# cserteGT3/RANSAC.jl

Measured on AMD Instinct MI355X. Metric: candidates_scored_per_sec, higher is better.
Workload: dtype f64; 1 GPU; cfg3: 10M-point 40-primitive cloud, 30% outliers, r=32 subsets, B=4096 candidates/GPU/step; points=10000000, subset_points=312500, score_mode=f64, parallelism=candidate-sharded x1, int32 sum all-reduce

## Files before the change

### include/ransac_hip_diag.h

```cpp
#ifndef RANSAC_HIP_DIAG_H
#define RANSAC_HIP_DIAG_H

#include "ransac_hip.h"

#ifdef __cplusplus
extern "C" {
#endif

int rh_dbg_cls_audit(rh_cloud *c, const rh_shape *shapes, int32_t b, const rh_params *p, double *out );
int rh_dbg_cls_soundness(rh_cloud *c, const rh_shape *shapes, int32_t b, const rh_params *p, uint64_t *out );
int rh_dbg_cls_soundness_tiles(rh_cloud *c, const rh_shape *shapes, int32_t b, const rh_params *p, uint64_t *out );
int rh_dbg_cls_soundness_nsig(rh_cloud *c, const rh_shape *shapes, int32_t b, const rh_params *p, uint64_t *out );
int rh_dbg_nsig(const rh_shape *shape, const rh_params *p, double M, double Nm, double Ln, int f32, uint32_t *mask_out ,
                const double *dirs, int64_t ndirs, int32_t *cells_out);
int rh_dbg_group_boxes(rh_cloud *c, double *out, int64_t cap, int64_t *ngroups_out);
int rh_dbg_kd_shape(int64_t s, int aligned, int64_t *info_out , int64_t *nodes_out, int64_t node_cap, int64_t *splits_out,
                    int64_t split_cap, int64_t *leaves_out, int64_t leaf_cap);
int rh_dbg_plane_order(rh_cloud *c, int64_t *info_out , double *sub_out, double *pl_out, int32_t *src_out, float *gb32_out,
                       uint32_t *gm32_out, uint64_t *en_out);
int rh_dbg_cylbox(const rh_shape *shape, const rh_params *p, double M, double Nm, int f32, const double *boxes, int64_t n,
                  uint8_t *skip_out, uint8_t *ball_out, float *fields_out );
int rh_dbg_cls_round(const rh_shape *shape, const rh_params *p, double M, double Nm, int f32, int64_t n, const double *xyz,
                     const double *nrm, float *ua_out, float *ub_out, float *rec_out , double *dbg4_out );
int rh_dbg_books2(const float *u2, int64_t nseq, int32_t *sure_count_out, uint64_t *sure_word_out, uint64_t *und_word_out,
                  uint8_t *any_und_out);
int rh_dbg_cls_u2(const rh_shape *shape, const rh_params *p, double M, double Nm, int f32, int64_t n, const double *xyz,
                  const double *nrm, float *u_out, float *u2_out, float *rec_out );
int rh_dbg_conebox(const rh_shape *shape, const rh_params *p, double M, double Nm, int f32, const double *boxes, int64_t n,
                   uint8_t *skip_out, float *fields_out );
int rh_dbg_cls_cone(const rh_shape *shape, const rh_params *p, double M, double Nm, int f32, int64_t n, const double *xyz,
                    const double *nrm, int device, float *ua_out, float *ub_out, uint8_t *near_out, float *rec_out ,
                    double *dbg4_out );
int rh_dbg_oct_search_selftest(int64_t n, uint64_t seed, int64_t queries, int64_t *mismatches);

int rh_dbg_enabled_events(const uint8_t *events, int64_t nseq, int32_t len, uint16_t *answers);

int rh_dbg_s4_stats(rh_cloud *c, int mode, uint64_t *out );

typedef struct { int64_t slot; int32_t level; int32_t pad; rh_shape shape; } rh_dbg_cand;
int rh_dbg_sample_fit(rh_cloud *c, const rh_params *p, uint64_t seed, int64_t k0, int32_t n_iters, const double *P_or_null,
                      int32_t rank, int32_t world, rh_dbg_cand *out, int32_t cap, int32_t *n_out, uint64_t *draws_out,
                      int32_t *gave_up_out, int32_t *info_out );

int rh_dbg_wave_keys(const uint32_t *keys, const uint8_t *act, const int32_t *slot, int32_t n, int32_t nslots, int u32, int device,
                     int32_t *sum_out , int32_t *minlead_out , int32_t *scal_out );

#ifdef __cplusplus
}
#endif
#endif
```

### ransac.jl_amd/_lib.py

```python
import ctypes as C
import os

_HERE = os.path.dirname(os.path.abspath(__file__))
SO_PATH = os.path.join(_HERE, "libransac_hip.so")
SO_PATH_DIAG = os.path.join(_HERE, "libransac_hip_diag.so")
OPTION_UNSET = -(1 << 63)
SCORE_PATH = {"auto": 0, "brute": 1, "groups": 2}
REFIT_PATH = {"auto": 0, "scan": 1, "culled": 2}

PLANE, SPHERE, CYLINDER, CONE = 0, 1, 2, 3
KIND_NAMES = {PLANE: "plane", SPHERE: "sphere", CYLINDER: "cylinder", CONE: "cone"}
SCORE_INT64_WRAP, SCORE_F64 = 0, 1
S_LENGTHC, S_ALLCAND, S_NOFMINSET = 1, 2, 3
RH_OK, RH_E_INVALID, RH_E_NODEVICE, RH_E_NOMEM, RH_E_CAPACITY, RH_E_INTERNAL = 0, -1, -2, -3, -4, -5


class Shape(C.Structure):
    _fields_ = [("kind", C.c_int32), ("outwards", C.c_int32), ("v", C.c_double * 10)]


class Params(C.Structure):
    _fields_ = [
        ("eps", C.c_double * 4), ("alpha", C.c_double * 4), ("cos_alpha", C.c_double * 4),
        ("collin_threshold", C.c_double), ("parallelthrdeg", C.c_double), ("cos_parallelthr", C.c_double),
# ... 200 lines not shown
    "rh_octree_info": (C.c_int, [_vp, _i32p, _i32p, _i32p]),
    "rh_octree_findleaf": (C.c_int, [_vp, _dp, _i32p]),
    "rh_octree_getnthcell": (C.c_int, [_vp, C.c_int32, C.c_int32, _i32p]),
    "rh_octree_node_info": (C.c_int, [_vp, C.c_int32, _dp, _dp, _i32p, _i32p, _i32p, C.POINTER(C.c_int64)]),
    "rh_octree_node_points": (C.c_int, [_vp, C.c_int32, C.POINTER(C.c_int64), C.c_int64]),
    "rh_octree_cell_enabled": (C.c_int, [_vp, _vp, C.c_int32, C.POINTER(C.c_int64), C.c_int64, C.POINTER(C.c_int64)]),
    "rh_set_option": (C.c_int, [_vp, C.c_char_p, C.c_int64]),
    "rh_get_option": (C.c_int, [_vp, C.c_char_p, _i64p, _i32p]),
    "rh_score_launch_info": (C.c_int, [_vp, C.POINTER(C.c_int32)]),
    "rh_last_list_launch_ms": (C.c_int, [_vp, C.POINTER(C.c_float)]),
    "rh_build_variant": (C.c_int, []),
    "rh_cloud_create_ms": (C.c_int, [_vp, _dp]),
    "rh_comm_unique_id": (C.c_int, [_vp]),
    "rh_comm_create": (C.c_int, [_vp, C.c_int32, C.c_int32, _vp, C.POINTER(_vp)]),
    "rh_comm_destroy": (C.c_int, [_vp]),
    "rh_score_batch_allreduce_dev": (C.c_int, [_vp, _vp, _vp, C.c_int32, C.c_int32, C.c_int32, _pp, _vp]),
    "rh_comm_fence": (C.c_int, [_vp, _vp]),
    "rh_comm_sync": (C.c_int, [_vp]),
    "rh_shape_extents": (C.c_int, [_vp, _sp, C.c_int32, _i64p, _i64p, C.POINTER(Extent)]),
    "rh_shape_extents_dev": (C.c_int, [_vp, _vp, C.c_int32, _vp, _vp, C.c_int64, _vp]),
    "rh_result_extents": (C.c_int, [_vp, C.POINTER(Result), C.POINTER(Extent)]),
    "rh_assign_points": (C.c_int, [_dp, _dp, C.c_int64, _sp, C.c_int32, _pp, C.c_int32, C.c_int, _i32p, _dp, _i64p, _i64p, _i64p]),
    "rh_assign_points_f32": (C.c_int, [C.POINTER(C.c_float), C.POINTER(C.c_float), C.c_int64, _sp, C.c_int32, _pp, C.c_int32, C.c_int,
                                       _i32p, _dp, _i64p, _i64p, _i64p]),
    "rh_cloud_assign": (C.c_int, [_vp, _sp, C.c_int32, _pp, C.c_int32, _i32p, _dp, _i64p, _i64p, _i64p]),
    "rh_cloud_assign_dev": (C.c_int, [_vp, _vp, C.c_int32, _pp, C.c_int32, _vp, _vp, _vp, _vp, _vp]),
    "rh_estimate_normals": (C.c_int, [_dp, C.c_int64, C.POINTER(NormalsParams), _dp, C.c_int, _dp, _dp, _i32p]),
    "rh_estimate_normals_f32": (C.c_int, [C.POINTER(C.c_float), C.c_int64, C.POINTER(NormalsParams), C.POINTER(C.c_float),
                                          C.c_int, C.POINTER(C.c_float), C.POINTER(C.c_float), _i32p]),
    "rh_cluster": (C.c_int, [_dp, C.c_int64, C.POINTER(ClusterParams), C.c_int, _i32p, _u8p, C.c_int64, _i64p, _i64p, _i64p, _i64p,
                             C.POINTER(ClusterStats)]),
    "rh_cluster_f32": (C.c_int, [C.POINTER(C.c_float), C.c_int64, C.POINTER(ClusterParams), C.c_int, _i32p, _u8p, C.c_int64, _i64p,
                                 _i64p, _i64p, _i64p, C.POINTER(ClusterStats)]),
    "rh_segment_smooth": (C.c_int, [_dp, _dp, _dp, C.c_int64, C.POINTER(SegmentParams), C.c_int, _i32p, _u8p, C.c_int64, _i64p, _i64p,
                                    _i64p, _i64p, C.POINTER(SegmentStats)]),
    "rh_segment_smooth_f32": (C.c_int, [C.POINTER(C.c_float), C.POINTER(C.c_float), C.POINTER(C.c_float), C.c_int64,
                                        C.POINTER(SegmentParams), C.c_int, _i32p, _u8p, C.c_int64, _i64p, _i64p, _i64p, _i64p,
                                        C.POINTER(SegmentStats)]),
    "rh_orient_normals": (C.c_int, [_dp, _dp, C.c_int64, C.POINTER(OrientParams), C.c_int, _dp, _i32p, _i32p, C.POINTER(OrientStats)]),
    "rh_orient_normals_f32": (C.c_int, [C.POINTER(C.c_float), C.POINTER(C.c_float), C.c_int64, C.POINTER(OrientParams), C.c_int,
                                        C.POINTER(C.c_float), _i32p, _i32p, C.POINTER(OrientStats)]),
    "rh_voxel_downsample": (C.c_int, [_dp, _dp, C.c_int64, C.POINTER(VoxelParams), C.c_int, _dp, _dp, _i64p, _i32p, C.c_int64,
                                      _i32p, _i64p, _i64p]),
    "rh_voxel_downsample_f32": (C.c_int, [C.POINTER(C.c_float), C.POINTER(C.c_float), C.c_int64, C.POINTER(VoxelParams), C.c_int,
                                          C.POINTER(C.c_float), C.POINTER(C.c_float), _i64p, _i32p, C.c_int64, _i32p, _i64p, _i64p]),
    "rh_knn": (C.c_int, [_dp, C.c_int64, C.c_int32, C.c_double, C.c_int, _i32p, _dp, _i32p]),
    "rh_knn_f32": (C.c_int, [C.POINTER(C.c_float), C.c_int64, C.c_int32, C.c_double, C.c_int, _i32p, _dp, _i32p]),
    "rh_knn_query": (C.c_int, [_dp, C.c_int64, _dp, C.c_int64, C.c_int32, C.c_double, C.c_int, _i32p, _dp, _i32p]),
    "rh_knn_query_f32": (C.c_int, [C.POINTER(C.c_float), C.c_int64, C.POINTER(C.c_float), C.c_int64, C.c_int32, C.c_double, C.c_int,
                                   _i32p, _dp, _i32p]),
    "rh_cloud_distance": (C.c_int, [_dp, _dp, C.c_int64, _dp, C.c_int64, C.POINTER(DistanceParams), C.c_int, _dp, _i32p,
                                    C.POINTER(DistanceStats)]),
    "rh_cloud_distance_f32": (C.c_int, [C.POINTER(C.c_float), C.POINTER(C.c_float), C.c_int64, C.POINTER(C.c_float), C.c_int64,
                                        C.POINTER(DistanceParams), C.c_int, _dp, _i32p, C.POINTER(DistanceStats)]),
    "rh_register": (C.c_int, [_dp, _dp, C.c_int64, _dp, C.c_int64, C.POINTER(RegisterParams), _dp, C.c_int, _dp,
                              C.POINTER(RegisterResult), _i32p, _dp]),
    "rh_register_f32": (C.c_int, [C.POINTER(C.c_float), C.POINTER(C.c_float), C.c_int64, C.POINTER(C.c_float), C.c_int64,
                                  C.POINTER(RegisterParams), _dp, C.c_int, _dp, C.POINTER(RegisterResult), _i32p, _dp]),
    "rh_describe": (C.c_int, [_dp, _dp, C.c_int64, C.c_int32, C.c_double, C.c_int, _u16p, _i32p]),
    "rh_describe_f32": (C.c_int, [C.POINTER(C.c_float), C.POINTER(C.c_float), C.c_int64, C.c_int32, C.c_double, C.c_int, _u16p,
                                  _i32p]),
    "rh_match_features": (C.c_int, [_u16p, C.c_int64, _u16p, C.c_int64, C.c_int32, C.c_int, _i32p, _u32p]),
    "rh_register_global": (C.c_int, [_dp, C.c_int64, _dp, C.c_int64, _i32p, _i32p, C.c_int64, C.POINTER(GlobalParams), _i32p,
                                     C.c_int, _dp, C.POINTER(GlobalResult), _i32p]),
    "rh_register_global_f32": (C.c_int, [C.POINTER(C.c_float), C.c_int64, C.POINTER(C.c_float), C.c_int64, _i32p, _i32p, C.c_int64,
                                         C.POINTER(GlobalParams), _i32p, C.c_int, _dp, C.POINTER(GlobalResult), _i32p]),
    "rh_remove_outliers": (C.c_int, [_dp, C.c_int64, C.POINTER(OutlierParams), C.c_int, _u8p, _i32p, C.c_int64, _i64p, _dp,
                                     C.POINTER(OutlierStats)]),
    "rh_remove_outliers_f32": (C.c_int, [C.POINTER(C.c_float), C.c_int64, C.POINTER(OutlierParams), C.c_int, _u8p, _i32p,
                                         C.c_int64, _i64p, _dp, C.POINTER(OutlierStats)]),
}

class DbgCand(C.Structure):
    _fields_ = [("slot", C.c_int64), ("level", C.c_int32), ("pad", C.c_int32), ("shape", Shape)]


DIAG_SIGNATURES = {
    "rh_dbg_sample_fit": (C.c_int, [_vp, _pp, C.c_uint64, C.c_int64, C.c_int32, _dp, C.c_int32, C.c_int32, C.POINTER(DbgCand),
                                    C.c_int32, _i32p, _u64p, _i32p, _i32p]),
    "rh_dbg_cls_audit": (C.c_int, [_vp, _sp, C.c_int32, _pp, _dp]),
    "rh_dbg_cls_soundness": (C.c_int, [_vp, _sp, C.c_int32, _pp, C.POINTER(C.c_uint64)]),
    "rh_dbg_cls_soundness_tiles": (C.c_int, [_vp, _sp, C.c_int32, _pp, C.POINTER(C.c_uint64)]),
    "rh_dbg_cls_soundness_nsig": (C.c_int, [_vp, _sp, C.c_int32, _pp, C.POINTER(C.c_uint64)]),
    "rh_dbg_nsig": (C.c_int, [_sp, _pp, C.c_double, C.c_double, C.c_double, C.c_int, C.POINTER(C.c_uint32), _dp, C.c_int64, _i32p]),
    "rh_dbg_group_boxes": (C.c_int, [_vp, _dp, C.c_int64, C.POINTER(C.c_int64)]),
    "rh_dbg_kd_shape": (C.c_int, [C.c_int64, C.c_int, _i64p, _i64p, C.c_int64, _i64p, C.c_int64, _i64p, C.c_int64]),
    "rh_dbg_plane_order": (C.c_int, [_vp, _i64p, _dp, _dp, _i32p, C.POINTER(C.c_float), C.POINTER(C.c_uint32), _u64p]),
    "rh_dbg_cylbox": (C.c_int, [_sp, _pp, C.c_double, C.c_double, C.c_int, _dp, C.c_int64, C.POINTER(C.c_uint8), C.POINTER(C.c_uint8), C.POINTER(C.c_float)]),
    "rh_dbg_cls_round": (C.c_int, [_sp, _pp, C.c_double, C.c_double, C.c_int, C.c_int64, _dp, _dp, C.POINTER(C.c_float), C.POINTER(C.c_float),
                                   C.POINTER(C.c_float), _dp]),
    "rh_dbg_books2": (C.c_int, [C.POINTER(C.c_float), C.c_int64, _i32p, _u64p, _u64p, _u8p]),
    "rh_dbg_cls_u2": (C.c_int, [_sp, _pp, C.c_double, C.c_double, C.c_int, C.c_int64, _dp, _dp, C.POINTER(C.c_float), C.POINTER(C.c_float),
                                C.POINTER(C.c_float)]),
    "rh_dbg_conebox": (C.c_int, [_sp, _pp, C.c_double, C.c_double, C.c_int, _dp, C.c_int64, C.POINTER(C.c_uint8), C.POINTER(C.c_float)]),
    "rh_dbg_cls_cone": (C.c_int, [_sp, _pp, C.c_double, C.c_double, C.c_int, C.c_int64, _dp, _dp, C.c_int, C.POINTER(C.c_float),
                                  C.POINTER(C.c_float), C.POINTER(C.c_uint8), C.POINTER(C.c_float), _dp]),
    "rh_dbg_oct_search_selftest": (C.c_int, [C.c_int64, C.c_uint64, C.c_int64, C.POINTER(C.c_int64)]),
    "rh_dbg_enabled_events": (C.c_int, [_u8p, C.c_int64, C.c_int32, C.POINTER(C.c_uint16)]),
    "rh_dbg_s4_stats": (C.c_int, [_vp, C.c_int, C.POINTER(C.c_uint64)]),
    "rh_dbg_wave_keys": (C.c_int, [C.POINTER(C.c_uint32), _u8p, _i32p, C.c_int32, C.c_int32, C.c_int, C.c_int, _i32p, _i32p, _i32p]),
}

_libs = {}


def variant():
    v = os.environ.get("RH_LIB_VARIANT", "product")
    if v not in ("product", "diag"):
        raise RuntimeError("RH_LIB_VARIANT=%r: expected 'product' or 'diag'" % v)
    return v


def _share_torch_hip_runtime():
    import sys
    if "torch" in sys.modules or os.environ.get("RH_SYSTEM_HIP"):
        return
    try:
        import importlib.util
        spec = importlib.util.find_spec("torch")
        if spec is None or not spec.submodule_search_locations:
            return
        path = os.path.join(list(spec.submodule_search_locations)[0], "lib", "libamdhip64.so")
        if os.path.exists(path):
            C.CDLL(path, mode=C.RTLD_GLOBAL)
    except (ImportError, OSError, ValueError):
        pass


def lib(which=None):
    which = which or variant()
    L = _libs.get(which)
    if L is None:
        path = SO_PATH if which == "product" else SO_PATH_DIAG
        if os.environ.get("RH_LIB_PATH"):
            path = os.environ["RH_LIB_PATH"]
        if not os.path.exists(path):
            raise RuntimeError(
                "%s is missing: the HIP extension has not been built and this package has no CPU "
                "fallback (build it with ransac.jl_amd/build.py)" % path)
        _share_torch_hip_runtime()
        L = C.CDLL(path)
        sigs = dict(SIGNATURES)
        if which == "diag":
            sigs.update(DIAG_SIGNATURES)
        for name, (res, args) in sigs.items():
            f = getattr(L, name, None)
            if f is None and os.environ.get("RH_LIB_PATH"):
                continue
            if f is None:
                raise AttributeError("%s does not export %s" % (path, name))
            f.restype = res
            f.argtypes = args
        if L.rh_build_variant() != (1 if which == "diag" else 0):
            raise RuntimeError("%s is not the %s build" % (path, which))
        _libs[which] = L
    return L


def check(rc):
    if rc != RH_OK:
        raise RansacHipError(rc, lib().rh_last_error().decode("utf-8", "replace"))
    return rc
```

### ransac.jl_amd/csrc/boxes32.hip

```cpp
#include "rh_internal.h"
#include "score_device.h"
#include "score4_device.h"
#include "score4_shared.h"

namespace {

using namespace rhdev;
using namespace rh4;

__global__ void gb32_kernel(const double *__restrict__ gb, int64_t gstride, int64_t ngroups, float *__restrict__ out)
{
    const int64_t g = (int64_t)blockIdx.x * blockDim.x + threadIdx.x;
    if (g >= ngroups) return;
    const double c[3] = { gb[g], gb[gstride + g], gb[2 * gstride + g] };
    const double h[3] = { gb[3 * gstride + g], gb[4 * gstride + g], gb[5 * gstride + g] };
    float o[8];
    box_to_f32(c, h, o);
#pragma unroll
    for (int k = 0; k < 8; k++) out[g * 8 + k] = o[k];
}

__global__ void st32_kernel(const double *__restrict__ gb, int64_t gstride, int64_t ngroups, int k_groups, int64_t nst, float *__restrict__ out)
{
    const int64_t st = (int64_t)blockIdx.x * blockDim.x + threadIdx.x;
    if (st >= nst) return;
    double lo[3] = { __builtin_inf(), __builtin_inf(), __builtin_inf() }, hi[3] = { -__builtin_inf(), -__builtin_inf(), -__builtin_inf() };
    bool bad = false;
    for (int64_t g = st * k_groups; g < (st + 1) * k_groups && g < ngroups; g++)
#pragma unroll
        for (int k = 0; k < 3; k++) {
            const double cc = gb[k * gstride + g], hh = gb[(3 + k) * gstride + g];
            bad |= !(fabs(cc) < __builtin_inf()) || !(fabs(hh) < __builtin_inf());
            lo[k] = fmin(lo[k], cc - hh);
            hi[k] = fmax(hi[k], cc + hh);
        }
    double c3[3], h3[3];
#pragma unroll
    for (int k = 0; k < 3; k++) {
        c3[k] = 0.5 * lo[k] + 0.5 * hi[k];
        h3[k] = fmax(hi[k] - c3[k], c3[k] - lo[k]) * 1.000000000001 + (fabs(lo[k]) + fabs(hi[k])) * 1e-15;
        bad |= !(fabs(c3[k]) < __builtin_inf()) || !(h3[k] < __builtin_inf());
    }
    float o[8];
    box_to_f32(c3, h3, o);
#pragma unroll
    for (int k = 0; k < 8; k++) out[st * 8 + k] = bad ? __builtin_nanf("") : o[k];
}

__global__ void __launch_bounds__(256)
nsig_kernel(const double *__restrict__ pts, int64_t stride, int64_t s, int64_t ngroups, uint32_t *__restrict__ out, unsigned long long *__restrict__ maxlen)
{
    __shared__ uint32_t m[4][4];
    const int lane = threadIdx.x & 63, wv = threadIdx.x >> 6;
    const int64_t g = (int64_t)blockIdx.x * 4 + wv;
    if (lane < 4) m[wv][lane] = 0u;
    __syncthreads();
    const int64_t i = g * 64 + lane;
    double len = 0.0;
    if (g < ngroups && i < s) {
        const double nx = pts[3 * stride + i], ny = pts[4 * stride + i], nz = pts[5 * stride + i];
        uint32_t w[3];
        nsig_point_bits(nx, ny, nz, w);
        if (w[0] != 0u) atomicOr(&m[wv][0], w[0]);
        if (w[1] != 0u) atomicOr(&m[wv][1], w[1]);
        if (w[2] != 0u) atomicOr(&m[wv][2], w[2]);
        const double l = sqrt((nx * nx + ny * ny) + nz * nz);
        if (l < __builtin_inf()) len = l;
    }
    unsigned long long lb = __builtin_bit_cast(unsigned long long, len);
    for (int off = 32; off > 0; off >>= 1) { const unsigned long long v = __shfl_down(lb, off); lb = v > lb ? v : lb; }
    if (lane == 0 && lb != 0ULL) atomicMax(maxlen, lb);
    __syncthreads();
    if (g < ngroups && lane < 4) out[g * 4 + lane] = m[wv][lane];
}

__global__ void nsig_st_kernel(const uint32_t *__restrict__ gm, int64_t ngroups, int k_groups, int64_t nst, uint32_t *__restrict__ out)
{
    const int64_t st = (int64_t)blockIdx.x * blockDim.x + threadIdx.x;
    if (st >= nst) return;
    uint32_t w[4] = { 0u, 0u, 0u, 0u };
    for (int64_t g = st * k_groups; g < (st + 1) * k_groups && g < ngroups; g++)
#pragma unroll
        for (int k = 0; k < 3; k++) w[k] |= gm[g * 4 + k];
#pragma unroll
    for (int k = 0; k < 4; k++) out[st * 4 + k] = w[k];
}

struct Twins32 {
    const double *pts;
    const double *gb;
    float *gb32, *st32, *tile32;
    uint32_t *gm32, *stm32;
};

int twins32_build(rh_cloud *c, const Twins32 &T, double *nrm_len)
{
    rhk_gb32_of(c, T.gb, c->ngroups, T.gb32);
    if (T.st32 != nullptr && c->nst > 0) rhk_runs32_of(c, T.gb, S4_STG, c->nst, T.st32);
    if (T.tile32 != nullptr && c->ntile > 0) rhk_runs32_of(c, T.gb, S4_TG, c->ntile, T.tile32);
    RH_HIP(hipGetLastError());
    if (nrm_len != nullptr) *nrm_len = 0.0;
    if (T.gm32 == nullptr || T.stm32 == nullptr || c->s <= 0) return RH_OK;
    rh_dev<unsigned long long> d_len;
    RH_TRY(d_len.alloc(1));
    RH_HIP(hipMemsetAsync(d_len, 0, sizeof(unsigned long long), c->stream));
    hipLaunchKernelGGL(nsig_kernel, dim3(cdiv4(c->ngroups, 4)), dim3(256), 0, c->stream, T.pts, c->s_pad, c->s, c->ngroups, T.gm32, d_len);
    hipLaunchKernelGGL(nsig_st_kernel, dim3(cdiv4(c->nst, 64)), dim3(64), 0, c->stream, T.gm32, c->ngroups, S4_STG, c->nst, T.stm32);
    RH_HIP(hipGetLastError());
    unsigned long long h_len = 0;
    if (nrm_len != nullptr) RH_HIP(hipMemcpyAsync(&h_len, d_len, sizeof h_len, hipMemcpyDeviceToHost, c->stream));
    RH_HIP(hipStreamSynchronize(c->stream));
    if (nrm_len != nullptr) *nrm_len = __builtin_bit_cast(double, h_len);
    return RH_OK;
}

}

void rhk_gb32_of(rh_cloud *c, const double *gb, int64_t ng, float *gb32)
{
    hipLaunchKernelGGL(gb32_kernel, dim3(cdiv4(ng, 256)), dim3(256), 0, c->stream, gb, c->ng_pad, ng, gb32);
}

void rhk_runs32_of(rh_cloud *c, const double *gb, int k, int64_t nruns, float *out)
{
    hipLaunchKernelGGL(st32_kernel, dim3(cdiv4(nruns, 64)), dim3(64), 0, c->stream, gb, c->ng_pad, c->ngroups, k, nruns, out);
}

int rhk_gb32_build(rh_cloud *c)
{
    if (c->ngroups == 0 || c->gb32 == nullptr) return RH_OK;
    return twins32_build(c, { c->sub, c->gb, c->gb32, c->st32, c->tile32, c->gm32, c->stm32 }, &c->nrm_len);
}

int rhk_plane_boxes(rh_cloud *c)
{
    if (c->pl_sub == nullptr || c->pl_gm32 == nullptr || c->pl_stm32 == nullptr || c->ngroups == 0) return RH_OK;
    rh_dev<double> gb;
    RH_TRY(gb.alloc(7 * c->ng_pad));
    RH_HIP(hipMemsetAsync(gb, 0, sizeof(double) * 7 * (size_t)c->ng_pad, c->stream));
    RH_HIP(hipMemsetAsync(c->pl_gb32, 0, sizeof(float) * 8 * (size_t)c->ng_pad, c->stream));
    RH_HIP(hipMemsetAsync(c->pl_gm32, 0, sizeof(uint32_t) * 4 * (size_t)c->ng_pad, c->stream));
    RH_TRY(rhk_group_bounds_of(c, c->pl_sub, c->s_pad, c->s, c->ngroups, gb, c->ng_pad));
    return twins32_build(c, { c->pl_sub, gb, c->pl_gb32, c->pl_st32, nullptr, c->pl_gm32, c->pl_stm32 }, nullptr);
}
```

### ransac.jl_amd/csrc/cloud.hip

```cpp
#include <functional>
#include <system_error>
#include <thread>
#include <stdarg.h>
#include <stdio.h>
#include <string.h>

#include <stdlib.h>

#include <algorithm>
#include <chrono>
#include <memory>
#include <new>
#include <utility>
#include <vector>

#include "rh_internal.h"
#include "score4_device.h"

static thread_local char g_err[512] = "";

void rh_set_error(const char *fmt, ...)
{
    va_list ap;
    va_start(ap, fmt);
// ... 204 lines not shown
    if (n < 0 || s < 0 || (n > 0 && (!xyz || !nrm)) || (s > 0 && !subset1)) {
        rh_set_error("rh_cloud_create: bad arguments (n=%lld s=%lld)", (long long)n, (long long)s);
        return RH_E_INVALID;
    }
    if (n > (int64_t)0x7FFFF000) { rh_set_error("clouds above 2^31 points are not supported"); return RH_E_INVALID; }
    for (int64_t j = 0; j < s; j++)
        if (subset1[j] < 1 || subset1[j] > n) {
            rh_set_error("subset index %lld at position %lld outside 1..%lld", (long long)subset1[j], (long long)j,
                         (long long)n);
            return RH_E_INVALID;
        }
    if (n > 2000000000LL) {
        rh_set_error("rh_cloud_create: %lld points exceed the 2e9 limit of one cloud", (long long)n);
        return RH_E_INVALID;
    }
    int ndev = 0;
    RH_TRY(rh_device_count(&ndev));
    if (ndev <= 0) { rh_set_error("no HIP device is visible; libransac_hip has no CPU fallback"); return RH_E_NODEVICE; }
    if (device < 0 || device >= ndev) { rh_set_error("device %d out of range (%d visible)", device, ndev); return RH_E_INVALID; }
    RH_HIP(hipSetDevice(device));
    const auto tc0 = std::chrono::steady_clock::now();
    auto ms_since = [](std::chrono::steady_clock::time_point t) { return std::chrono::duration<double, std::milli>(std::chrono::steady_clock::now() - t).count(); };
    double ms_kd = 0, ms_before_kd = 0;
    const bool prof = rh_opt_on(nullptr, RH_OPT_CREATE_PROF);
    double t_prev = 0;

    rh_cloud *c = new (std::nothrow) rh_cloud();
    if (!c) { rh_set_error("out of host memory"); return RH_E_NOMEM; }
    rh_opt_init_cloud(c);
    c->device = device;
    c->n = n;
    c->s = s;
    c->n_pad = ((n + RH_SC_TILE - 1) / RH_SC_TILE) * RH_SC_TILE;
    c->s_pad = ((s + RH_SC_TILE - 1) / RH_SC_TILE) * RH_SC_TILE;
    if (c->n_pad == 0) c->n_pad = RH_SC_TILE;
    if (c->s_pad == 0) c->s_pad = RH_SC_TILE;
    c->nwords = (n + 63) / 64;
    c->swords = (s + 63) / 64;
    c->nblocks = (c->nwords + RH_WORDS_PER_BLOCK - 1) / RH_WORDS_PER_BLOCK;
    c->dis_stride = c->s_pad + RH_SC_TILE;

    int rc = RH_OK;
    rh_dev<double> t_xyz, t_nrm;
    std::unique_ptr<int32_t[]> h_idx_own;
    int32_t *h_idx = nullptr;
    auto stamp = [&](const char *what) {
        if (!prof) return;
        if (c->stream) (void)hipStreamSynchronize(c->stream);
        const double t = ms_since(tc0);
        fprintf(stderr, "[rh_cloud_create] %-28s %8.2f ms\n", what, t - t_prev);
        t_prev = t;
    };
    auto fail = [&](int code) {
        cloud_free(c);
        return code;
    };
#define CK(x) do { rc = (x); if (rc != RH_OK) return fail(rc); } while (0)
#define CKH(x) do { hipError_t e_ = (x); if (e_ != hipSuccess) { rh_set_error("%s: %s", #x, hipGetErrorString(e_)); return fail(RH_E_NODEVICE); } } while (0)
    CKH(hipStreamCreateWithFlags(&c->own_stream, hipStreamNonBlocking));
    c->stream = c->own_stream;
    CKH(hipEventCreate(&c->ev0));
    CKH(hipEventCreate(&c->ev1));
    for (int k = 0; k < 5; k++) CKH(hipEventCreate(&c->evk[k]));
    CKH(hipStreamCreateWithFlags(&c->copy_stream, hipStreamNonBlocking));
    CKH(hipEventCreateWithFlags(&c->ev_copied, hipEventDisableTiming));
    CKH(hipEventCreateWithFlags(&c->ev_sync, hipEventDisableTiming));
    CK(c->full.alloc(6 * c->n_pad));
    CK(c->rec.alloc(8 * std::max<int64_t>(n, 1)));
    CK(c->sel_list.alloc(c->nwords * 64 + 64));
    CK(c->sub.alloc(6 * c->s_pad));
    CK(c->dis.alloc(6 * c->dis_stride));
    CK(c->sub_idx0.alloc(s));
    CK(c->sub_perm.alloc(c->s_pad));
    CKH(hipMemsetAsync(c->sub_perm, 0, sizeof(int32_t) * (size_t)std::max<int64_t>(c->s_pad, 1), c->stream));
    c->ngroups = (s + 63) / 64;
    c->ng_pad = ((c->ngroups + RH_G2_TG - 1) / RH_G2_TG) * RH_G2_TG + RH_G2_TG;
    CK(c->gb.alloc(7 * c->ng_pad));
    CK(c->gb32.alloc(8 * c->ng_pad));
    c->nst = (c->ngroups + RH_S4_STG - 1) / RH_S4_STG;
    CK(c->st32.alloc(8 * std::max<int64_t>(1, c->nst)));
    c->ntile = (c->ngroups + RH_G2_TG - 1) / RH_G2_TG;
    CK(c->tile32.alloc(8 * std::max<int64_t>(1, c->ntile)));
    CK(c->gm32.alloc(4 * c->ng_pad));
    CK(c->stm32.alloc(4 * std::max<int64_t>(1, c->nst)));
    CK(c->dis_gb.alloc(7 * c->ng_pad));
    CK(c->dis_gb32.alloc(8 * c->ng_pad));
    CKH(hipMemsetAsync(c->dis_gb, 0, sizeof(double) * 7 * (size_t)c->ng_pad, c->stream));
    CKH(hipMemsetAsync(c->gb, 0, sizeof(double) * 7 * (size_t)c->ng_pad, c->stream));
    {
        const int64_t e = rh_opt_int(nullptr, RH_OPT_SCORE_PATH, RH_SCORE_PATH_AUTO);
        c->use_groups = s >= RH_G2_MIN_POINTS;
        if (e == RH_SCORE_PATH_BRUTE) c->use_groups = false;
        if (e == RH_SCORE_PATH_GROUPS) c->use_groups = s > 0;
        c->kd_aligned = kd_aligned_for(s, rh_opt_int(nullptr, RH_OPT_KD_ALIGN, 0));
    }
    CK(rhk_enabled_alloc(c));
    CK(c->refit_mask.alloc(c->nwords));
    CK(c->idx_out.alloc(n));
    CK(c->d_nk.alloc(4));
    CK(c->ws[0].d_nk2.alloc(8));
    CKH(hipMemsetAsync(c->full, 0, sizeof(double) * 6 * (size_t)c->n_pad, c->stream));
    CKH(hipMemsetAsync(c->sub, 0, sizeof(double) * 6 * (size_t)c->s_pad, c->stream));
    CKH(hipMemsetAsync(c->dis, 0, sizeof(double) * 6 * (size_t)c->dis_stride, c->stream));
    stamp("streams, allocations, memsets");

    if (n > 0) {
        CK(t_xyz.alloc(3 * n));
        CK(t_nrm.alloc(3 * n));
        CKH(hipMemcpyAsync(t_xyz, xyz, sizeof(double) * 3 * (size_t)n, hipMemcpyHostToDevice, c->stream));
        CKH(hipMemcpyAsync(t_nrm, nrm, sizeof(double) * 3 * (size_t)n, hipMemcpyHostToDevice, c->stream));
        stamp("upload (xyz, nrm)");
        CK(rhk_transpose_aos(c, t_xyz, t_nrm, n, nullptr, n, c->full, c->n_pad));
        CK(rhk_pack_records(c, t_xyz, t_nrm, n, c->rec));
        stamp("AoS -> SoA, records");
        if (rh_opt_on(nullptr, RH_OPT_AABB_HOST)) cloud_aabb(xyz, n, c->k_lo, &c->k_size, &c->k_mag);
        else CK(cloud_aabb_device(c, t_xyz, xyz, n));
        stamp("bounding box");
        CK(rhk_korder_build(c, t_xyz, t_nrm, c->k_lo, c->k_size, c->k_mag));
        stamp("Morton order of the cloud");
        if (s > 0) {
            h_idx_own.reset(new (std::nothrow) int32_t[2 * (size_t)s]);
            h_idx = h_idx_own.get();
            if (!h_idx) { rh_set_error("out of host memory"); return fail(RH_E_NOMEM); }
            ms_before_kd = ms_since(tc0);
            const auto tkd0 = std::chrono::steady_clock::now();
            const bool ord_morton = rh_opt_on(nullptr, RH_OPT_SUB_ORDER);
            const bool kd_device = !rh_opt_on(nullptr, RH_OPT_KD_HOST) && !ord_morton;
            if (kd_device) {
                for (int64_t j = 0; j < s; j++) h_idx[j] = (int32_t)(subset1[j] - 1);
                rh_dev<int32_t> d_idx_in;
                CK(d_idx_in.alloc(s));
                CKH(hipMemcpyAsync(d_idx_in, h_idx, sizeof(int32_t) * (size_t)s, hipMemcpyHostToDevice, c->stream));
                CK(rhk_kd_order(c, t_xyz, t_nrm, d_idx_in));
                d_idx_in.reset();
                ms_kd = ms_since(tkd0);
                CK(rhk_transpose_aos(c, t_xyz, t_nrm, n, c->sub_idx0, s, c->sub, c->s_pad));
                CK(rhk_group_bounds(c));
            } else {
            double lo[3] = { 0, 0, 0 }, hi[3] = { 0, 0, 0 }, mag = 0;
            bool first = true;
            for (int64_t j = 0; j < s; j++) {
                const double *pp = xyz + 3 * (subset1[j] - 1);
                for (int k = 0; k < 3; k++) {
                    const double v = pp[k];
                    if (!(v == v) || v - v != 0) continue;
                    if (first || v < lo[k]) lo[k] = v;
                    if (first || v > hi[k]) hi[k] = v;
                    if (fabs(v) > mag) mag = fabs(v);
                }
                first = false;
            }
            c->coord_mag = mag;
            double nmag = 0;
            for (int64_t j = 0; j < s; j++) {
                const double *nn = nrm + 3 * (subset1[j] - 1);
                for (int k = 0; k < 3; k++) {
                    const double v = fabs(nn[k]);
                    if (v - v == 0 && v > nmag) nmag = v;
                }
            }
            c->nrm_mag = nmag;
            std::vector<int32_t> order((size_t)s);
            for (int64_t j = 0; j < s; j++) order[(size_t)j] = (int32_t)j;
            if (ord_morton) {
                std::vector<std::pair<uint64_t, int32_t>> keys((size_t)s);
                for (int64_t j = 0; j < s; j++) {
// ... 718 lines not shown
```

### ransac.jl_amd/csrc/kdorder.hip

```cpp
#include <stdlib.h>

#include <algorithm>
#include <vector>

#include <hipcub/hipcub.hpp>

#include "rh_internal.h"
#ifdef RH_DIAG
#include "ransac_hip_diag.h"
#endif

namespace {

inline unsigned cdivq(int64_t a, int64_t b) { return (unsigned)((a + b - 1) / b); }

__device__ __forceinline__ uint32_t ord32(float v)
{
    const uint32_t b = __builtin_bit_cast(uint32_t, v);
    if ((b & 0x7fffffffu) > 0x7f800000u) return 0xffffffffu;
    return (b & 0x80000000u) ? ~b : (b | 0x80000000u);
}
__device__ __forceinline__ float unord32(uint32_t u)
{
    const uint32_t b = (u & 0x80000000u) ? (u & 0x7fffffffu) : ~u;
// ... 334 lines not shown
            levels.push_back(cur);
            std::vector<KdNode> nxt;
            nxt.reserve(cur.size() * 2);
            for (const KdNode &nd : cur) {
                const int32_t cnt = nd.hi - nd.lo;
                if (cnt <= 64) { nxt.push_back(nd); continue; }
                const int32_t nl = (int32_t)kd_left_count(cnt, c->kd_aligned);
                nxt.push_back(KdNode{ nd.lo, nd.lo + nl });
                nxt.push_back(KdNode{ nd.lo + nl, nd.hi });
            }
            cur.swap(nxt);
        }
    }
    size_t max_seg = 1;
    for (const auto &lv : levels) max_seg = std::max(max_seg, lv.size());
    RH_TRY(pf.alloc(3 * s));
    RH_TRY(ord[0].alloc(s));
    RH_TRY(ord[1].alloc(s));
    RH_TRY(keys[0].alloc(s));
    RH_TRY(keys[1].alloc(s));
    RH_TRY(box.alloc(6 * (int64_t)max_seg));
    RH_TRY(mags.alloc(2));
    RH_HIP(hipMemsetAsync(mags, 0, sizeof(unsigned long long) * 2, c->stream));
    float *px = pf, *py = pf + s, *pz = pf + 2 * s;
    const dim3 gs(cdivq(s, 256)), blk(256);
    hipLaunchKernelGGL(kd_gather_kernel, gs, blk, 0, c->stream, d_xyz, d_nrm, d_idx0, s, px, py, pz, ord[0], mags);
    RH_HIP(hipGetLastError());
    RH_HIP(hipcub::DeviceRadixSort::SortPairs(nullptr, tmp_bytes, keys[0].get(), keys[1].get(), ord[0].get(), ord[1].get(), (int)s, 0, 64, c->stream));
    RH_TRY(tmp.alloc((int64_t)tmp_bytes));
    std::vector<int32_t> h_lo;
    std::vector<uint8_t> h_act;
    std::vector<size_t> off_lo, off_act;
    for (const auto &lv : levels) {
        off_lo.push_back(h_lo.size());
        off_act.push_back(h_act.size());
        for (const KdNode &nd : lv) { h_lo.push_back(nd.lo); h_act.push_back(nd.hi - nd.lo > 64 ? 1 : 0); }
        h_lo.push_back((int32_t)s);
    }
    RH_TRY(seg_lo.alloc((int64_t)h_lo.size()));
    RH_TRY(seg_act.alloc((int64_t)h_act.size()));
    if (!h_lo.empty()) RH_HIP(hipMemcpyAsync(seg_lo, h_lo.data(), sizeof(int32_t) * h_lo.size(), hipMemcpyHostToDevice, c->stream));
    if (!h_act.empty()) RH_HIP(hipMemcpyAsync(seg_act, h_act.data(), h_act.size(), hipMemcpyHostToDevice, c->stream));
    int cur = 0;
    for (size_t L = 0; L < levels.size(); L++) {
        const int nseg = (int)levels[L].size();
        const int32_t *lo_l = seg_lo + off_lo[L];
        const uint8_t *act_l = seg_act + off_act[L];
        hipLaunchKernelGGL(kd_fill_box_kernel, dim3(cdivq((int64_t)nseg * 6, 256)), blk, 0, c->stream, box, nseg);
        hipLaunchKernelGGL(kd_box_kernel, gs, blk, 0, c->stream, px, py, pz, ord[cur], s, lo_l, act_l, nseg, box);
        hipLaunchKernelGGL(kd_key_kernel, gs, blk, 0, c->stream, px, py, pz, ord[cur], s, lo_l, act_l, nseg, box, keys[0]);
        RH_HIP(hipGetLastError());
        int seg_bits = 1;
        while ((1 << seg_bits) < nseg) seg_bits++;
        RH_HIP(hipcub::DeviceRadixSort::SortPairs(tmp.get(), tmp_bytes, keys[0].get(), keys[1].get(), ord[cur].get(), ord[cur ^ 1].get(), (int)s, 0, 32 + seg_bits, c->stream));
        cur ^= 1;
    }
    hipLaunchKernelGGL(kd_finish_kernel, gs, blk, 0, c->stream, ord[cur], d_idx0, s, c->sub_perm, c->sub_idx0);
    RH_HIP(hipGetLastError());
    unsigned long long h_mags[2] = { 0, 0 };
    RH_HIP(hipMemcpyAsync(h_mags, mags, sizeof h_mags, hipMemcpyDeviceToHost, c->stream));
    RH_HIP(hipStreamSynchronize(c->stream));
    c->coord_mag = __builtin_bit_cast(double, h_mags[0]);
    c->nrm_mag = __builtin_bit_cast(double, h_mags[1]);
    return RH_OK;
}

int rhk_plane_order_build(rh_cloud *c)
{
    if (!c->use_groups || c->s <= 0 || c->nst <= 0) return RH_OK;
    if (c->s > (int64_t)0x7fffffff) { rh_set_error("rhk_plane_order_build: subset of %lld points", (long long)c->s); return RH_E_INVALID; }
    std::vector<int32_t> lo;
    kd_walk(c->s, c->kd_aligned, PO_ST, [&](int64_t a, int64_t, int64_t) { lo.push_back((int32_t)a); });
    lo.push_back((int32_t)c->s);
    const int64_t nblk = (int64_t)lo.size() - 1;
    rh_dev<int32_t> d_lo;
    RH_TRY(d_lo.alloc((int64_t)lo.size()));
    RH_HIP(hipMemcpyAsync(d_lo, lo.data(), sizeof(int32_t) * lo.size(), hipMemcpyHostToDevice, c->stream));
    RH_TRY(c->pl_sub.alloc(6 * c->s_pad));
    RH_TRY(c->pl_src.alloc(c->s_pad));
    RH_TRY(c->pl_st32.alloc(8 * c->nst));
    RH_TRY(c->pl_stm32.alloc(4 * c->nst));
    RH_TRY(c->pl_gb32.alloc(8 * c->ng_pad));
    RH_TRY(c->pl_gm32.alloc(4 * c->ng_pad));
    RH_TRY(c->pl_enabled.alloc(c->swords));
    RH_HIP(hipMemsetAsync(c->pl_sub, 0, sizeof(double) * 6 * (size_t)c->s_pad, c->stream));
    RH_HIP(hipMemsetAsync(c->pl_src, 0, sizeof(int32_t) * (size_t)c->s_pad, c->stream));
    hipLaunchKernelGGL(plane_order_kernel, dim3((unsigned)nblk), dim3(PO_THREADS), 0, c->stream, c->sub, c->s_pad, d_lo.get(), c->pl_src.get());
    hipLaunchKernelGGL(plane_gather_kernel, dim3(cdivq(c->s, 256)), dim3(256), 0, c->stream, c->sub, c->s_pad, c->s, c->pl_src.get(), c->pl_sub.get());
    RH_HIP(hipGetLastError());
    return rhk_plane_boxes(c);
}

int rhk_plane_enabled_sync(rh_cloud *c)
{
    if (c->pl_enabled == nullptr || c->s <= 0) return RH_OK;
    hipLaunchKernelGGL(plane_enabled_kernel, dim3(cdivq(c->swords * 64, 256)), dim3(256), 0, c->stream, c->sub_enabled, c->s, c->swords,
                       c->pl_src.get(), c->pl_enabled.get());
    RH_HIP(hipGetLastError());
    return RH_OK;
}

#ifdef RH_DIAG
extern "C" int rh_dbg_kd_shape(int64_t s, int aligned, int64_t *info_out, int64_t *nodes_out, int64_t node_cap, int64_t *splits_out,
                               int64_t split_cap, int64_t *leaves_out, int64_t leaf_cap)
{
    if (info_out == nullptr || s < 1 || s > (int64_t)0x7fffffff || aligned < -1 || aligned > 1) { rh_set_error("rh_dbg_kd_shape: bad arguments"); return RH_E_INVALID; }
    const bool al = aligned < 0 ? kd_aligned_for(s, rh_opt_int(nullptr, RH_OPT_KD_ALIGN, 0)) : aligned != 0;
    int64_t nn = 0, ns = 0, nl = 0;
    kd_walk(s, al, RH_KD_NODE, [&](int64_t lo, int64_t hi, int64_t mid) {
        if (mid == 0) {
            if (nodes_out != nullptr && nn < node_cap) { nodes_out[2 * nn] = lo; nodes_out[2 * nn + 1] = hi; }
            nn++;
        } else {
            if (splits_out != nullptr && ns < split_cap) { splits_out[3 * ns] = lo; splits_out[3 * ns + 1] = mid; splits_out[3 * ns + 2] = hi; }
            ns++;
        }
    });
    if (leaves_out != nullptr)
        kd_walk(s, al, 64, [&](int64_t lo, int64_t hi, int64_t mid) {
            if (mid != 0) return;
            if (nl < leaf_cap) { leaves_out[2 * nl] = lo; leaves_out[2 * nl + 1] = hi; }
            nl++;
        });
    int64_t depth = 0;
    for (std::vector<int64_t> cur(1, s); ; depth++) {
        std::vector<int64_t> nxt;
        for (int64_t cnt : cur)
            if (cnt > 64) { const int64_t l = kd_left_count(cnt, al); nxt.push_back(l); nxt.push_back(cnt - l); }
        if (nxt.empty()) break;
        std::sort(nxt.begin(), nxt.end());
        nxt.erase(std::unique(nxt.begin(), nxt.end()), nxt.end());
        cur.swap(nxt);
    }
    info_out[0] = nn; info_out[1] = ns; info_out[2] = nl; info_out[3] = depth; info_out[4] = al ? 1 : 0;
    return RH_OK;
}

extern "C" int rh_dbg_plane_order(rh_cloud *c, int64_t *info_out, double *sub_out, double *pl_out, int32_t *src_out, float *gb32_out,
                                  uint32_t *gm32_out, uint64_t *en_out)
{
    if (c == nullptr || info_out == nullptr) { rh_set_error("rh_dbg_plane_order: bad arguments"); return RH_E_INVALID; }
    const bool has = c->pl_sub != nullptr;
    info_out[0] = c->s; info_out[1] = c->ngroups; info_out[2] = c->nst; info_out[3] = has ? 1 : 0;
    if (!has || c->s <= 0) return RH_OK;
    RH_HIP(hipSetDevice(c->device));
    const size_t s = (size_t)c->s;
    for (int k = 0; k < 6; k++) {
        if (sub_out != nullptr) RH_HIP(hipMemcpyAsync(sub_out + k * s, c->sub + k * c->s_pad, sizeof(double) * s, hipMemcpyDeviceToHost, c->stream));
        if (pl_out != nullptr) RH_HIP(hipMemcpyAsync(pl_out + k * s, c->pl_sub + k * c->s_pad, sizeof(double) * s, hipMemcpyDeviceToHost, c->stream));
    }
    if (src_out != nullptr) RH_HIP(hipMemcpyAsync(src_out, c->pl_src, sizeof(int32_t) * s, hipMemcpyDeviceToHost, c->stream));
    if (gb32_out != nullptr) RH_HIP(hipMemcpyAsync(gb32_out, c->pl_gb32, sizeof(float) * 8 * (size_t)c->ngroups, hipMemcpyDeviceToHost, c->stream));
    if (gm32_out != nullptr) RH_HIP(hipMemcpyAsync(gm32_out, c->pl_gm32, sizeof(uint32_t) * 4 * (size_t)c->ngroups, hipMemcpyDeviceToHost, c->stream));
    if (en_out != nullptr) {
        RH_HIP(hipMemcpyAsync(en_out, c->sub_enabled, sizeof(uint64_t) * (size_t)c->swords, hipMemcpyDeviceToHost, c->stream));
        RH_HIP(hipMemcpyAsync(en_out + c->swords, c->pl_enabled, sizeof(uint64_t) * (size_t)c->swords, hipMemcpyDeviceToHost, c->stream));
    }
    RH_HIP(hipStreamSynchronize(c->stream));
    return RH_OK;
}
#endif
```

### ransac.jl_amd/csrc/options.cpp

```cpp
#include <stdlib.h>
#include <string.h>

#include "rh_internal.h"

namespace {

enum { T_INT = 0, T_FLAG = 1, T_ENUM_SCORE = 2, T_ENUM_REFIT = 3, T_ENUM_ORDER = 4 };

struct OptDef {
    int id;
    const char *key;
#ifdef RH_DIAG
    const char *env;
#endif
    int type;
};

#ifdef RH_DIAG
#define RH_O(id, key, env, type) { id, key, env, type }
#else
#define RH_O(id, key, env, type) { id, key, type }
#endif

const OptDef kDefs[] = {
    RH_O(RH_OPT_SCORE_PATH, "score_path", "RH_SCORE_PATH", T_ENUM_SCORE),
    RH_O(RH_OPT_S4_ROWS, "s4_rows", "RH_S4_R", T_INT),
    RH_O(RH_OPT_UNP_WORDS, "unp_words", "RH_UNP_WORDS", T_INT),
    RH_O(RH_OPT_ST_CULL, "st_cull", "RH_ST_CULL", T_INT),
    RH_O(RH_OPT_REFIT_PATH, "refit_path", "RH_REFIT_PATH", T_ENUM_REFIT),
    RH_O(RH_OPT_BATCHES_IN_FLIGHT, "batches_in_flight", "RH_BATCHES_IN_FLIGHT", T_INT),
    RH_O(RH_OPT_ST_LIST_MB, "st_list_mb", "RH_ST_LIST_MB", T_INT),
    RH_O(RH_OPT_NSIG, "nsig", "RH_NSIG", T_INT),
    RH_O(RH_OPT_PLANE_ORDER, "plane_order", "RH_PLANE_ORDER", T_INT),
    RH_O(RH_OPT_KD_ALIGN, "kd_align", "RH_KD_ALIGN", T_INT),
#ifdef RH_DIAG
    RH_O(RH_OPT_CREATE_PROF, "create_prof", "RH_CREATE_PROF", T_FLAG),
    RH_O(RH_OPT_AABB_HOST, "aabb_host", "RH_AABB_HOST", T_FLAG),
    RH_O(RH_OPT_SUB_ORDER, "sub_order", "RH_SUB_ORDER", T_ENUM_ORDER),
    RH_O(RH_OPT_KD_HOST, "kd_host", "RH_KD_HOST", T_FLAG),
    RH_O(RH_OPT_NO_SPREAD, "no_spread", "RH_NO_SPREAD", T_FLAG),
    RH_O(RH_OPT_OCT_CHAIN_W, "oct_chain_w", "RH_OCT_CHAIN_W", T_INT),
    RH_O(RH_OPT_NO_MANAGED_STORE, "no_managed_store", "RH_NO_MANAGED_STORE", T_FLAG),
    RH_O(RH_OPT_OCT_ONE_WINDOW, "oct_one_window", "RH_OCT_ONE_WINDOW", T_FLAG),
    RH_O(RH_OPT_OCT_WINDOW_ITERS, "oct_window_iters", "RH_OCT_WINDOW_ITERS", T_INT),
    RH_O(RH_OPT_NO_FUSED_SCORE, "no_fused_score", "RH_NO_FUSED_SCORE", T_FLAG),
    RH_O(RH_OPT_NO_PIPELINE, "no_pipeline", "RH_NO_PIPELINE", T_FLAG),
    RH_O(RH_OPT_NO_OCT_CHAIN, "no_oct_chain", "RH_NO_OCT_CHAIN", T_FLAG),
    RH_O(RH_OPT_REFIT_BLOCKS, "refit_blocks", "RH_REFIT_BLOCKS", T_INT),
    RH_O(RH_OPT_NO_FUSED_SAMPLER, "no_fused_sampler", "RH_NO_FUSED_SAMPLER", T_FLAG),
    RH_O(RH_OPT_NO_CREC, "no_crec", "RH_NO_CREC", T_FLAG),
    RH_O(RH_OPT_LONG_WINDOW_SETS, "long_window_sets", "RH_LONG_WINDOW_SETS", T_INT),
    RH_O(RH_OPT_NO_OCT_TAB, "no_oct_tab", "RH_NO_OCT_TAB", T_FLAG),
    RH_O(RH_OPT_NO_DRIVER_CACHE, "no_driver_cache", "RH_NO_DRIVER_CACHE", T_FLAG),
    RH_O(RH_OPT_HOST_SAMPLER, "host_sampler", "RH_HOST_SAMPLER", T_FLAG),
    RH_O(RH_OPT_DRIVER_PROF, "driver_prof", "RH_DRIVER_PROF", T_FLAG),
    RH_O(RH_OPT_G2_DBG, "g2_dbg", "RH_G2_DBG", T_INT),
    RH_O(RH_OPT_KREFIT_DBG, "krefit_dbg", "RH_KREFIT_DBG", T_FLAG),
    RH_O(RH_OPT_NO_FAST_EXTRACT, "no_fast_extract", "RH_NO_FAST_EXTRACT", T_FLAG),
#endif
};
constexpr int kNDefs = (int)(sizeof(kDefs) / sizeof(kDefs[0]));

int64_t g_opt[RH_OPT_COUNT];
bool g_init = false;

void init_once()
{
    if (g_init) return;
    for (int i = 0; i < RH_OPT_COUNT; i++) g_opt[i] = RH_OPTION_UNSET;
    g_init = true;
}

const OptDef *find_key(const char *key)
{
    if (key == nullptr) return nullptr;
    for (int i = 0; i < kNDefs; i++)
        if (strcmp(kDefs[i].key, key) == 0) return &kDefs[i];
    return nullptr;
}

#ifdef RH_DIAG
int64_t parse_env(const OptDef &d, const char *e)
{
    switch (d.type) {
    case T_FLAG: return 1;
    case T_ENUM_SCORE: return e[0] == 'b' ? RH_SCORE_PATH_BRUTE : (e[0] == 'g' ? RH_SCORE_PATH_GROUPS : RH_OPTION_UNSET);
    case T_ENUM_REFIT: return e[0] == 's' ? RH_REFIT_PATH_SCAN : (e[0] == 'c' ? RH_REFIT_PATH_CULLED : RH_OPTION_UNSET);
    case T_ENUM_ORDER: return e[0] == 'm' ? 1 : 0;
    default: return (int64_t)atoll(e);
    }
}
#endif

}

int64_t rh_opt(const rh_cloud *c, int id)
{
    if (id < 0 || id >= RH_OPT_COUNT) return RH_OPTION_UNSET;
    init_once();
    if (c != nullptr && c->opt[id] != RH_OPTION_UNSET) return c->opt[id];
    if (g_opt[id] != RH_OPTION_UNSET) return g_opt[id];
#ifdef RH_DIAG
    for (int i = 0; i < kNDefs; i++)
        if (kDefs[i].id == id) {
            const char *e = getenv(kDefs[i].env);
            return e != nullptr ? parse_env(kDefs[i], e) : RH_OPTION_UNSET;
        }
#endif
    return RH_OPTION_UNSET;
}

#ifdef RH_DIAG
const char *rh_opt_env_string(const char *name) { return getenv(name); }
#endif

void rh_opt_init_cloud(rh_cloud *c)
{
    for (int i = 0; i < RH_OPT_COUNT; i++) c->opt[i] = RH_OPTION_UNSET;
}

extern "C" int rh_build_variant(void)
{
#ifdef RH_DIAG
    return 1;
#else
    return 0;
#endif
}

extern "C" int rh_set_option(rh_cloud *c, const char *key, int64_t value)
{
    init_once();
    const OptDef *d = find_key(key);
    if (d == nullptr) { rh_set_error("rh_set_option: unknown option '%s'", key ? key : "(null)"); return RH_E_INVALID; }
    if (value != RH_OPTION_UNSET) {
        bool ok = true;
        switch (d->id) {
        case RH_OPT_SCORE_PATH: ok = value >= 0 && value <= RH_SCORE_PATH_GROUPS; break;
        case RH_OPT_REFIT_PATH: ok = value >= 0 && value <= RH_REFIT_PATH_CULLED; break;
        case RH_OPT_S4_ROWS: ok = value == 0 || value == 1 || value == 2 || value == 4 || value == 8 || value == 12 || value == 16; break;
        case RH_OPT_UNP_WORDS: ok = value >= 0 && value <= 16384; break;
        case RH_OPT_ST_CULL: ok = value >= 0 && value <= 2; break;
        case RH_OPT_BATCHES_IN_FLIGHT: ok = value >= 0 && value <= RH_MAX_IN_FLIGHT; break;
        case RH_OPT_ST_LIST_MB: ok = value >= 0 && value <= (1 << 20); break;
        case RH_OPT_NSIG: ok = value == 0 || value == 2; break;
        case RH_OPT_PLANE_ORDER: ok = value >= 0 && value <= 2; break;
        case RH_OPT_KD_ALIGN: ok = value >= 0 && value <= 2; break;
        default: break;
        }
        if (!ok) { rh_set_error("rh_set_option: value %lld is not valid for '%s'", (long long)value, key); return RH_E_INVALID; }
    }
    if (d->id == RH_OPT_SCORE_PATH && c != nullptr) {
        rh_set_error("rh_set_option: 'score_path' is fixed when a cloud is created (its point order depends on it): set it process-wide (cloud = NULL) before rh_cloud_create");
        return RH_E_INVALID;
    }
    if (d->id == RH_OPT_KD_ALIGN && c != nullptr) {
        rh_set_error("rh_set_option: 'kd_align' is fixed when a cloud is created (it shapes the cloud's internal point order): set it process-wide (cloud = NULL) before rh_cloud_create");
        return RH_E_INVALID;
    }
    if (c != nullptr) {
        if (d->id == RH_OPT_BATCHES_IN_FLIGHT) { const int rc = rh_cloud_join(c); if (rc != RH_OK) return rc; }
        c->opt[d->id] = value;
    } else {
        g_opt[d->id] = value;
    }
    return RH_OK;
}

extern "C" int rh_get_option(const rh_cloud *c, const char *key, int64_t *value_out, int32_t *is_set)
{
    const OptDef *d = find_key(key);
    if (d == nullptr || value_out == nullptr) { rh_set_error("rh_get_option: unknown option '%s'", key ? key : "(null)"); return RH_E_INVALID; }
    const int64_t v = rh_opt(c, d->id);
    *value_out = v == RH_OPTION_UNSET ? 0 : v;
    if (is_set != nullptr) *is_set = v != RH_OPTION_UNSET;
    return RH_OK;
}
```

### ransac.jl_amd/csrc/rh_internal.h

```cpp
#pragma once

#include <hip/hip_runtime.h>
#include <stdint.h>

#include <vector>

#include "ransac_hip.h"
#include "dev_buf.h"
#include "enabled_state.h"

void rh_set_error(const char *fmt, ...);

#define RH_HIP(call)                                                                        \
    do {                                                                                    \
        hipError_t e_ = (call);                                                             \
        if (e_ != hipSuccess) {                                                             \
            rh_set_error("%s failed: %s (%s:%d)", #call, hipGetErrorString(e_), __FILE__,   \
                         __LINE__);                                                         \
            return RH_E_NODEVICE;                                                           \
        }                                                                                   \
    } while (0)

#define RH_TRY(call)                 \
    do {                             \
        int rc_ = (call);            \
        if (rc_ != RH_OK) return rc_; \
    } while (0)

static inline int cdiv(int64_t a, int64_t b) { return (int)((a + b - 1) / b); }

enum rh_opt_id {
    RH_OPT_SCORE_PATH = 0,
    RH_OPT_S4_ROWS,
    RH_OPT_UNP_WORDS,
    RH_OPT_ST_CULL,
    RH_OPT_REFIT_PATH,
    RH_OPT_BATCHES_IN_FLIGHT,
    RH_OPT_ST_LIST_MB,
    RH_OPT_NSIG,
    RH_OPT_PLANE_ORDER,
    RH_OPT_KD_ALIGN,
    RH_OPT_N_PRODUCT,
    RH_OPT_CREATE_PROF = RH_OPT_N_PRODUCT, RH_OPT_AABB_HOST, RH_OPT_SUB_ORDER, RH_OPT_KD_HOST, RH_OPT_NO_SPREAD, RH_OPT_OCT_CHAIN_W,
    RH_OPT_NO_MANAGED_STORE, RH_OPT_OCT_ONE_WINDOW, RH_OPT_OCT_WINDOW_ITERS, RH_OPT_NO_FUSED_SCORE, RH_OPT_NO_PIPELINE,
    RH_OPT_NO_OCT_CHAIN, RH_OPT_REFIT_BLOCKS, RH_OPT_NO_FUSED_SAMPLER, RH_OPT_NO_CREC, RH_OPT_LONG_WINDOW_SETS, RH_OPT_NO_OCT_TAB,
    RH_OPT_NO_DRIVER_CACHE, RH_OPT_HOST_SAMPLER, RH_OPT_DRIVER_PROF, RH_OPT_G2_DBG, RH_OPT_KREFIT_DBG, RH_OPT_NO_FAST_EXTRACT,
    RH_OPT_COUNT
};
struct rh_cloud;
int64_t rh_opt(const rh_cloud *c, int id);
void rh_opt_init_cloud(rh_cloud *c);
#ifdef RH_DIAG
const char *rh_opt_env_string(const char *name);
static inline bool rh_opt_on(const rh_cloud *c, int id) { const int64_t v = rh_opt(c, id); return v != RH_OPTION_UNSET && v != 0; }
static inline int64_t rh_opt_int(const rh_cloud *c, int id, int64_t dflt) { const int64_t v = rh_opt(c, id); return v == RH_OPTION_UNSET ? dflt : v; }
#else
static inline bool rh_opt_on(const rh_cloud *c, int id) { if (id >= RH_OPT_N_PRODUCT) return false; const int64_t v = rh_opt(c, id); return v != RH_OPTION_UNSET && v != 0; }
static inline int64_t rh_opt_int(const rh_cloud *c, int id, int64_t dflt) { if (id >= RH_OPT_N_PRODUCT) return dflt; const int64_t v = rh_opt(c, id); return v == RH_OPTION_UNSET ? dflt : v; }
#endif

struct rh_prep {
    double f[12];
};

__host__ __device__ inline void prep_derived(rh_prep &o, int kind)
{
    o.f[11] = (((((fabs(o.f[0]) + fabs(o.f[1])) + fabs(o.f[2])) + fabs(o.f[3])) + fabs(o.f[4])) + fabs(o.f[5])) + fabs(o.f[6]);
    if (kind == RH_CYLINDER) {
        const double a2 = (o.f[0] * o.f[0] + o.f[1] * o.f[1]) + o.f[2] * o.f[2];
        const double k = 2.0 - a2;
        o.f[8] = (1.0 + fabs(o.f[3])) + (fabs(o.f[4]) + fabs(o.f[5]));
        o.f[9] = k;
        o.f[10] = 1.0 + fabs(k) * a2;
    }
}

__host__ __device__ __forceinline__ void prep_one(const rh_shape &s, rh_prep &o)
{
#pragma unroll
    for (int i = 0; i < 12; i++) o.f[i] = 0.0;
    const double sgn = s.outwards ? 1.0 : -1.0;
    switch (s.kind) {
    case RH_PLANE: {
        for (int i = 0; i < 6; i++) o.f[i] = s.v[i];
        const double a = s.v[3], b = s.v[4], c = s.v[5];
        const double inv = 1.0 / sqrt((a * a + b * b) + c * c);
        o.f[6] = inv * a; o.f[7] = inv * b; o.f[8] = inv * c;
        break;
    }
    case RH_SPHERE:
        for (int i = 0; i < 4; i++) o.f[i] = s.v[i];
        o.f[4] = sgn;
        break;
    case RH_CYLINDER:
        for (int i = 0; i < 7; i++) o.f[i] = s.v[i];
        o.f[7] = sgn;
        break;
    default:
        for (int i = 0; i < 6; i++) o.f[i] = s.v[i];
        o.f[6] = s.v[7];
        o.f[7] = s.v[8];
        o.f[8] = sgn;
        break;
    }
    prep_derived(o, s.kind);
}
inline void rh_prep_host(const rh_shape &s, rh_prep *out) { prep_one(s, *out); }

struct rh_prepf {
    float f[12];
};
template <int KIND>
__host__ __device__ inline rh_prepf prepf_of(const rh_prep &P)
{
    rh_prepf o;
    for (int i = 0; i < 9; i++) o.f[i] = (float)P.f[i];
    for (int i = 9; i < 12; i++) o.f[i] = 0.0f;
    if (KIND == RH_PLANE) {
        const float a = o.f[3], b = o.f[4], c = o.f[5];
        const float inv = 1.0f / sqrtf((a * a + b * b) + c * c);
        o.f[6] = inv * a; o.f[7] = inv * b; o.f[8] = inv * c;
    }
    if (KIND == RH_SPHERE) { o.f[5] = o.f[6] = o.f[7] = o.f[8] = 0.0f; }
    if (KIND == RH_CYLINDER) { o.f[8] = 0.0f; }
// ... 63 lines not shown
    int64_t mstride4 = 0;
    bool masks4 = false;
    rh_dev<uint16_t> d_stlist;
    rh_dev<int32_t> d_stcount;
    int64_t stlist_cap = 0, stlist_nst = 0;
    int64_t stlist_nomem = 0;
    rh_dev<uint64_t> d_segmask;
    int64_t segmask_words = 0;
};
struct rh_bins {
    const rh_prep *prep[4];
    const int32_t *orig[4];
    const void *cls[4];
    const float *box[4];
};
static inline rh_bins rh_bins_at(const rh_prep *prep, const int32_t *orig, const void *cls, const float *box, const int64_t off[4])
{
    rh_bins B;
    for (int k = 0; k < 4; k++) {
        B.prep[k] = prep + off[k];
        B.orig[k] = orig + off[k];
        B.cls[k] = cls ? (const char *)cls + (size_t)off[k] * 64 : nullptr;
        B.box[k] = box ? box + off[k] : nullptr;
    }
    return B;
}
static inline rh_bins rh_ws_bins(const rh_batch_ws &w)
{
    const int64_t off[4] = { 0, w.batch_cap, 2 * w.batch_cap, 3 * w.batch_cap };
    return rh_bins_at(w.d_prep, w.d_orig, w.d_qpre, w.d_box, off);
}
struct rh_score_job {
    rh_bins bins = {};
    int64_t bstride = 0;
    const uint64_t *en[4] = { nullptr, nullptr, nullptr, nullptr };
    const int32_t *nk[4] = { nullptr, nullptr, nullptr, nullptr };
    int32_t bound = 0;
    int32_t kind_bound[4] = { 0, 0, 0, 0 };
    const double *eps = nullptr, *cosa = nullptr;
    int32_t *d_counts = nullptr;
    uint64_t *d_masks_int = nullptr;
    rh_s4_points points = { nullptr, 0, 0, 0, nullptr };
    const int32_t *stop = nullptr;
    bool open_count = false;
    hipEvent_t ev_listed = nullptr;
};
struct rh_cloud {
    int64_t opt[RH_OPT_COUNT];
    int device = -1;
    hipStream_t stream = nullptr;
    hipStream_t own_stream = nullptr;
    hipEvent_t ev0 = nullptr, ev1 = nullptr;
    hipEvent_t evk[5] = { nullptr, nullptr, nullptr, nullptr, nullptr };
    hipStream_t copy_stream = nullptr;
    hipEvent_t ev_copied = nullptr;
    hipEvent_t ev_sync = nullptr;
    int64_t n = 0, s = 0;
    int64_t n_pad = 0, s_pad = 0;
    int64_t nwords = 0, swords = 0;
    int64_t nblocks = 0;

    rh_dev<double> full;
    rh_dev<double> set_ws;
    rh_dev<int32_t> set_level;
    int64_t set_ws_sets = 0;
    rh_dev<double> rec;
    rh_dev<double> sub;
    rh_dev<int32_t> sub_idx0;
    rh_dev<int32_t> sub_perm;
    rh_dev<double> gb;
    int64_t ngroups = 0, ng_pad = 0;
    double create_ms[4] = { 0, 0, 0, 0 };
    double coord_mag = 0;
    double nrm_mag = 0;
    bool use_groups = false;
    bool kd_aligned = false;
    rh_dev<float> gb32;
    rh_dev<float> st32;
    int64_t nst = 0;
    rh_dev<float> tile32;
    int64_t ntile = 0;
    rh_dev<uint32_t> gm32;
    rh_dev<uint32_t> stm32;
    double nrm_len = 0;
    rh_dev<double> pl_sub;
    rh_dev<int32_t> pl_src;
    rh_dev<float> pl_gb32;
    rh_dev<uint32_t> pl_gm32;
    rh_dev<float> pl_st32;
    rh_dev<uint32_t> pl_stm32;
    rh_dev<uint64_t> pl_enabled;
    rh_dev<double> dis_gb;

    rh_enabled_state en;
    rh_dev<uint64_t> enabled;
    rh_dev<uint64_t> sub_enabled;
    rh_dev<double> dis;
    int64_t dis_stride = 0;
    rh_dev<int32_t> d_ndis;
    int64_t n_dis = 0;
    rh_dev<uint64_t> oct_men;
    rh_dev<int32_t> oct_prefix;
    rh_dev<int32_t> en_block_sums;
    rh_dev<int32_t> word_prefix;
    rh_dev<int32_t> sel_list;
    rh_dev<double> crec;
    rh_dev<int32_t> block_sums;
    rh_dev<int32_t> d_total;

    bool k_built = false;
    double k_lo[3] = { 0, 0, 0 }, k_size = 1;
    double k_mag = 0;
    rh_dev<double> fullk;
    rh_dev<float> fullk32;
    rh_dev<double> kgb;
    int64_t kg_pad = 0;
    rh_dev<int32_t> klist;
    rh_dev<int32_t> kctr;
    rh_dev<uint8_t> kflag;
    bool oct_built = false;
    int oct_depth = 0, oct_max_depth = 0;
    rh_dev<uint64_t> oct_code;
    rh_dev<int32_t> oct_perm;
    rh_dev<int32_t> oct_pos;
    rh_dev<rh_oct_state> oct_state;
    rh_dev<float> dis_gb32;
    rh_dev<unsigned long long> s4_stats;
    rh_dev<int32_t> oct_adv_tab;
    rh_dev<unsigned long long> oct_adv_bits;
    int64_t oct_adv_cells = 0;
    rh_dev<double> oct_adv_E;
    rh_dev<uint64_t> oct_code_o;
    rh_dev<int32_t> oct_tab;
    int oct_tab_level = 0;
    rh_dev<double> oct_P;
    std::vector<uint64_t> h_oct_code;
    std::vector<int32_t> h_oct_perm, h_oct_pos;

    rh_dev<uint64_t> refit_mask;
    rh_dev<int64_t> idx_out;

    double comp_beta = 0;
    int32_t comp_conn26 = 1;
    rh_dev<char> comp_tab;
    int64_t comp_cap = 0;
    rh_dev<uint64_t> comp_scal;
    rh_pinned<uint64_t> comp_h;

    rh_dev<double> ext_part;
    int64_t ext_part_rows = 0;
    rh_dev<int32_t> ext_flag;
    rh_dev<char> ext_in;

    rh_dev<char> asg_ws;
    rh_dev<char> asg_io;

    rh_batch_ws ws[RH_MAX_IN_FLIGHT];
    uint32_t pipe_k = 0;

    rh_dev<int32_t> d_nk;
    rh_dev<uint64_t> d_masks;
    rh_dev<int32_t> d_zero;
    hipEvent_t ev_cull = nullptr;
    float last_cull_ms = 0.f;
    int32_t last_s4[4] = { 0, 0, 0, 0 };

    rh_dev<int64_t> d_ranks;

    bool f32 = false;
    bool f32_groups = false;
    rh_dev<float> full32;
// ... 188 lines not shown
```

### ransac.jl_amd/csrc/score4.hip

```cpp
#include <stdio.h>
#include <stdlib.h>

#include <vector>

#include "rh_internal.h"
#include "score_device.h"
#include "score4_device.h"
#include "score4_shared.h"
#include "wave_keys.h"

namespace {

using namespace rhdev;
using namespace rh4;

constexpr int S4_GB = 2;
constexpr unsigned S4_GM = (1u << S4_GB) - 1u;
constexpr int S4_ROW = 65;
constexpr int S4_W = 4;
template <int R, bool MASK = false, bool LIST = false>
struct S4Shared {
    static_assert(S4_TG == (1 << S4_GB) && R * 64 * S4_TG <= 65536 && (R % S4_W == 0 || R < S4_W), "entry encoding: S4_GB bits of group, the rest of 16 for the candidate");
    rh_f32x4 pa[S4_TG][S4_ROW];
    rh_f32x2 pb[S4_TG][S4_ROW];
    uint64_t len[S4_TG];
    rh_f32x4 gbox[S4_TG][2];
    rh_u32x4 gmask[S4_TG];
    uint16_t plist[R * 64 * S4_TG + 2];
    uint16_t ctab[LIST ? R * 64 : 2];
    int32_t cntb[S4_W][64];
    unsigned long long maskb[S4_W][64];
    uint16_t qb[S4_W][128];
    int weirdw[S4_TG];
    int npairs, next_batch;
};

struct S4KindArgs {
    const rh_cls *cls;
    const float *box;
    const rh_prep *prep;
    const int32_t *orig, *nk;
    const uint64_t *en;
    double eps, cosa;
    const double *pts;
    int64_t stride;
    const float *gb32;
    const uint32_t *gm32;
};
struct S4AllArgs {
    const int32_t *stop;
    int row0;
    int rows;
    S4KindArgs k[4];
    int64_t ntiles, bstride, ngroups;
    uint64_t *masks;
    uint8_t *occ;
    int64_t mstride;
    unsigned long long *stats;
    const uint16_t *stlist;
    const int32_t *stcount;
    int64_t stcap;
};

#ifdef RH_DIAG
#define S4_STAT(stats, idx, val) do { const unsigned long long v_ = (unsigned long long)(val); if ((stats) != nullptr && (threadIdx.x & 63) == 0) atomicAdd((stats) + (idx), v_); } while (0)
#else
#define S4_STAT(stats, idx, val) do { } while (0)
#endif

#define RH4_CONST_AS __attribute__((address_space(4)))

static __device__ __forceinline__ int wave_shr1(int v) { return __builtin_amdgcn_update_dpp(0, v, 0x138, 0xf, 0xf, false); }
static __device__ __forceinline__ int wave_shl1(int v) { return __builtin_amdgcn_update_dpp(0, v, 0x130, 0xf, 0xf, false); }

static __device__ __forceinline__ int run_total(int v, int key, int lane)
{
    static_assert(S4_TG <= 4, "two steps cover runs of four");
    const int k1 = wave_shr1(key), u1 = wave_shr1(v);
    v += (lane >= 1 && k1 == key) ? u1 : 0;
    const int k2 = wave_shr1(k1), u2 = wave_shr1(wave_shr1(v));
    v += (lane >= 2 && k2 == key) ? u2 : 0;
    const int kn = wave_shl1(key);
    return (lane == 63 || kn != key) ? v : 0;
}

template <int KIND, int R, bool MASK, bool F32, bool LIST>
static __device__ __forceinline__ void
score4_batch(S4Shared<R, MASK, LIST> &sh, const int wv, const int lane, const int head, const int n, const int cbase, const double *__restrict__ pts,
             int64_t stride, const int64_t p0, const rh_prep *__restrict__ prep, const rh_cls *__restrict__ cls,
             const int32_t *__restrict__ orig, double eps, double cosa, int32_t *__restrict__ counts, const bool weird,
             uint64_t *__restrict__ masks, uint8_t *__restrict__ occ, const int64_t mstride, const int64_t g0, unsigned long long *__restrict__ stats)
{
    (void)stats;
    S4_STAT(stats, 24 * KIND + 8, 1);
    const bool act = lane < n;
    const uint32_t e = sh.plist[head + (act ? lane : 0)];
    const int g = (int)(e & S4_GM), ci = LIST ? (int)sh.ctab[e >> S4_GB] : cbase + (int)(e >> S4_GB);
    const rh_f32x4 *__restrict__ rowa = &sh.pa[g][0];
    const rh_f32x2 *__restrict__ rowb = &sh.pb[g][0];
    const rh_cls *__restrict__ rec = &cls[ci];
    int total = 0;
    uint64_t word = 0;
    int qbh = 0, qbn = 0;
    auto drain_b = [&](int k) {
        wave_lds_sync();
        const bool on = lane < k;
        const unsigned e2 = on ? sh.qb[wv][(qbh + lane) & 127] : 0u;
        const int slot = (int)(e2 >> 6);
        const uint32_t pe = sh.plist[head + slot];
        const int64_t gi = p0 + (int)(pe & S4_GM) * 64 + (int)(e2 & 63u);
        uint64_t r;
        if (F32) {
            const rh_prepf Pv = prepf_of<KIND>(prep[LIST ? (int)sh.ctab[pe >> S4_GB] : cbase + (int)(pe >> S4_GB)]);
            const rh_f32x4 a = sh.pa[pe & S4_GM][e2 & 63u];
            const rh_f32x2 b = sh.pb[pe & S4_GM][e2 & 63u];
            r = test_point<KIND>(Pv, a.x, a.y, a.z, a.w, b.x, b.y, eps, cosa);
        } else {
            const rh_prep Pv = prep[LIST ? (int)sh.ctab[pe >> S4_GB] : cbase + (int)(pe >> S4_GB)];
            r = test_point<KIND>(Pv, pts[gi], pts[stride + gi], pts[2 * stride + gi], pts[3 * stride + gi], pts[4 * stride + gi],
                                 pts[5 * stride + gi], eps, cosa);
        }
        S4_STAT(stats, 24 * KIND + (k == 64 ? 11 : 12), 1);
        S4_STAT(stats, 24 * KIND + 13, __popcll(r & (k >= 64 ? ~0ULL : ((1ULL << k) - 1ULL))));
        if (on && ((r >> lane) & 1ULL)) {
            atomicAdd(&sh.cntb[wv][slot], 1);
            if (MASK) atomicOr(&sh.maskb[wv][slot], 1ULL << (e2 & 63u));
        }
        qbh = (qbh + k) & 127;
        qbn -= k;
    };
    if (KIND != RH_CONE) {
        constexpr int NF = KIND == RH_PLANE ? 9 : (KIND == RH_SPHERE ? 8 : 11);
        rh_cls C;
#pragma unroll
        for (int f = 0; f < NF; f++) C.f[f] = rec->f[f];
        const bool exact_only = weird || is_nan_bits(rec->f[RH_CLS_FLAG]);
// ... 83 lines not shown
        total = sh.cntb[wv][lane] + __popcll(sure);
        if (MASK) word = sh.maskb[wv][lane] | sure;
    }
    if (MASK) {
        const bool nz = act && word != 0;
        const uint64_t nzm = WB(nz);
        if (nzm != 0) {
            const int keyp = wave_shr1(act ? ci : -1 - lane);
            const uint64_t starts = WB(lane == 0 || keyp != (act ? ci : -1 - lane));
            const uint64_t below = lane == 63 ? ~0ULL : ((2ULL << lane) - 1ULL);
            const int rs = 63 - __builtin_clzll(starts & below);
            const uint64_t after = lane == 63 ? 0ULL : (starts >> (lane + 1));
            const int re = after != 0 ? lane + __builtin_ctzll(after) : 63;
            const uint64_t runm = (re == 63 ? ~0ULL : ((2ULL << re) - 1ULL)) & ~((1ULL << rs) - 1ULL);
            const int tot = __popcll(nzm & runm);
            int base = 0;
            int64_t mrow = 0;
            if (nz || (lane == rs && tot > 0)) mrow = orig[ci];
            if (lane == rs && tot > 0) base = atomicAdd((int32_t *)occ + mrow, tot);
            base = __shfl(base, rs);
            if (nz) {
                const int rank = __popcll(nzm & runm & ((1ULL << lane) - 1ULL));
                rh_u64x2 ent;
                ent.x = (uint64_t)(g0 + g);
                ent.y = word;
                ((rh_u64x2 *)masks)[mrow * mstride + base + rank] = ent;
            }
        }
    }
    S4_STAT(stats, 24 * KIND + 14, __popcll(WB(act && total > 0)));
    const int v = run_total(act ? total : 0, act ? ci : -1 - lane, lane);
    if (v != 0) atomicAdd(&counts[orig[ci]], v);
}

template <int KIND, int R, bool MASK, bool F32, bool LIST>
static __device__ __forceinline__ void
score4_segment(S4Shared<R, MASK, LIST> &sh, const S4KindArgs &K, const int32_t *__restrict__ nkp, const uint16_t *__restrict__ list, const int64_t bstride, const int lo, const int hi,
               const double *__restrict__ pts, int64_t stride, const int64_t g0, const unsigned live, const bool weird,
               int32_t *__restrict__ counts, int dbg, uint64_t *__restrict__ masks, uint8_t *__restrict__ occ, const int64_t mstride,
               unsigned long long *__restrict__ stats)
{
    (void)stats;
    const int lane = threadIdx.x & 63;
    const int wv = __builtin_amdgcn_readfirstlane(threadIdx.x >> 6);
    const int nk = *nkp;
    S4_STAT(stats, 24 * KIND + 0, 1);
    constexpr int NB = S4Fields<KIND>::NBOX;
    constexpr int CPW = (R + S4_W - 1) / S4_W;
    float B[2][RH_BOX_FIELDS];
    int slot[LIST ? CPW : 1];
    auto clamped = [&](int h) { const int ci = ((lo + wv + h * S4_W) << 6) + lane; return (lo + wv + h * S4_W < hi && ci < nk) ? ci : 0; };
    if (LIST) {
#pragma unroll
        for (int h = 0; h < CPW; h++) slot[h] = (int)list[clamped(h)];
#pragma unroll
        for (int h = 0; h < CPW; h++) {
            const int ci = ((lo + wv + h * S4_W) << 6) + lane;
            if (lo + wv + h * S4_W < hi && ci < nk) sh.ctab[ci - (lo << 6)] = (uint16_t)slot[h];
        }
    }
    {
        const int cil = LIST ? slot[0] : clamped(0);
#pragma unroll
        for (int f = 0; f < NB; f++) B[0][f] = K.box[(int64_t)f * bstride + cil];
    }
#pragma unroll
    for (int h = 0; h < CPW; h++) {
        const int c = lo + wv + h * S4_W;
        if (c >= hi) break;
        const int ci = (c << 6) + lane;
        if (h + 1 < CPW) {
            const int cinl = LIST ? slot[h + 1 < CPW ? h + 1 : 0] : clamped(h + 1);
#pragma unroll
            for (int f = 0; f < NB; f++) B[(h + 1) & 1][f] = K.box[(int64_t)f * bstride + cinl];
        }
        unsigned surv = 0;
#pragma unroll
        for (int g = 0; g < S4_TG; g++) {
            const rh_f32x4 g0v = sh.gbox[g][0], g1v = sh.gbox[g][1];
            rh_box32 G;
            G.cx = g0v.x; G.cy = g0v.y; G.cz = g0v.z; G.hx = g0v.w; G.hy = g1v.x; G.hz = g1v.y; G.hr = g1v.z;
            bool skip = box_skip32<KIND>(B[h & 1], G);
            if (KIND == RH_PLANE) skip |= !nsig_meet(B[h & 1], sh.gmask[g]);
            surv |= skip ? 0u : (1u << g);
        }
        if (dbg == 2) surv = (1u << S4_TG) - 1u;
        surv &= live;
        if (ci >= nk || dbg == 1) surv = 0;
        const int k = __popc(surv);
        const uint64_t b0 = WB(k & 1), b1 = WB(k & 2), b2 = WB(k & 4), b3 = WB(k & 8);
        const int tot = __popcll(b0) + 2 * __popcll(b1) + 4 * __popcll(b2) + 8 * __popcll(b3);
        S4_STAT(stats, 24 * KIND + 1 + (h < 3 ? h : 3), 1);
        S4_STAT(stats, 24 * KIND + 5, __popcll(WB(ci < nk)));
        S4_STAT(stats, 24 * KIND + 7, tot);
        if (tot == 0) { S4_STAT(stats, 24 * KIND + 6, 1); continue; }
        int base = 0;
        if (lane == 0) base = atomicAdd(&sh.npairs, tot);
        base = __builtin_amdgcn_readfirstlane(base);
        auto mb = [&](uint64_t m) { return __builtin_amdgcn_mbcnt_hi((uint32_t)(m >> 32), __builtin_amdgcn_mbcnt_lo((uint32_t)m, 0)); };
        int pos = base + mb(b0) + 2 * mb(b1) + 4 * mb(b2) + 8 * mb(b3);
#pragma unroll
        for (int g = 0; g < S4_TG; g++) {
            const bool on = (surv >> g) & 1u;
            sh.plist[on ? pos : R * 64 * S4_TG] = (uint16_t)(((ci - (lo << 6)) << S4_GB) | g);
            pos += on ? 1 : 0;
        }
    }
    __syncthreads();
    const int npairs = sh.npairs;
    for (;;) {
        int bt = 0;
        if (lane == 0) bt = atomicAdd(&sh.next_batch, 1);
        bt = __builtin_amdgcn_readfirstlane(bt);
        if (bt * 64 >= npairs) break;
        score4_batch<KIND, R, MASK, F32, LIST>(sh, wv, lane, bt * 64, min(64, npairs - bt * 64), lo << 6, pts, stride, g0 * 64, K.prep, K.cls, K.orig,
                                         K.eps, K.cosa, counts, weird, masks, occ, mstride, g0, stats);
    }
}

template <class SH>
static __device__ __forceinline__ void s4_stage(SH &sh, const double *__restrict__ pts, int64_t stride, int64_t s,
                                                const uint64_t *__restrict__ enabled_words, const int64_t p0, const float *__restrict__ gb32,
                                                const uint32_t *__restrict__ gm32, const int64_t ngroups)
{
    static_assert(S4_TG % S4_W == 0, "every wave stages S4_TG / S4_W groups");
    const int tid = threadIdx.x, lane = tid & 63;
    const int wv = __builtin_amdgcn_readfirstlane(tid >> 6);
    constexpr int GPW = S4_TG / S4_W;
    double x[GPW], y[GPW], z[GPW], nx[GPW], ny[GPW], nz[GPW];
#pragma unroll
    for (int q = 0; q < GPW; q++) {
        const int64_t gi = p0 + (int64_t)(wv + q * S4_W) * 64 + lane;
        x[q] = pts[gi]; y[q] = pts[stride + gi]; z[q] = pts[2 * stride + gi];
        nx[q] = pts[3 * stride + gi]; ny[q] = pts[4 * stride + gi]; nz[q] = pts[5 * stride + gi];
    }
#pragma unroll
    for (int q = 0; q < GPW; q++) {
        const int g = wv + q * S4_W;
        const int64_t gi = p0 + (int64_t)g * 64 + lane;
        uint64_t v = valid_mask((gi >> 6) << 6, s);
        if (enabled_words != nullptr && v != 0) v &= enabled_words[gi >> 6];
        const bool on = (v >> (gi & 63)) & 1ULL;
        rh_f32x4 a = { 0.f, 0.f, 0.f, 0.f };
        rh_f32x2 b = { 0.f, 0.f };
        bool bad = false;
        if (on) {
            a.x = (float)x[q]; a.y = (float)y[q]; a.z = (float)z[q]; a.w = (float)nx[q]; b.x = (float)ny[q]; b.y = (float)nz[q];
            const float sum = (fabsf(a.x) + fabsf(a.y)) + (fabsf(a.z) + fabsf(a.w)) + (fabsf(b.x) + fabsf(b.y));
            bad = !(sum < __builtin_inff());
        }
        sh.pa[g][lane] = a;
        sh.pb[g][lane] = b;
        const uint64_t wb = WB(bad);
        if (lane == 0) { sh.weirdw[g] = wb != 0 ? 1 : 0; sh.len[g] = v; }
    }
    if (tid == 0) { sh.npairs = 0; sh.next_batch = 0; }
    if (tid < 2 * S4_TG) {
        const int64_t g = p0 / 64 + (tid >> 1);
        sh.gbox[tid >> 1][tid & 1] = ((const rh_f32x4 *)gb32)[(g < ngroups ? g : ngroups - 1) * 2 + (tid & 1)];
    }
    if (tid >= 64 && tid < 64 + S4_TG) {
        const int64_t g = p0 / 64 + (tid - 64);
        rh_u32x4 m = { 0xffffffffu, 0xffffffffu, 0xffffffffu, 0u };
        if (gm32 != nullptr) m = ((const rh_u32x4 *)gm32)[g < ngroups ? g : ngroups - 1];
        sh.gmask[tid - 64] = m;
    }
}

template <int R, bool MASK, bool F32, bool TAIL = false, bool LIST = false>
#ifndef RH_S4_MINBLK
#define RH_S4_MINBLK 7
#endif
__global__ void __launch_bounds__(64 * S4_W, (F32 && !(LIST && R == 16)) ? 8 : RH_S4_MINBLK)
score4_kernel(int64_t s, const S4AllArgs A, int32_t *__restrict__ counts, int dbg_arg)
{
#ifdef RH_DIAG
    const int dbg = dbg_arg;
#else
    constexpr int dbg = 0;
    (void)dbg_arg;
#endif
    __shared__ S4Shared<R, MASK, LIST> sh;
    int64_t tile = blockIdx.x;
    int rowy = (int)blockIdx.y;
    if (!TAIL && A.rows > 0) {
        const int64_t k = blockIdx.x >> 3;
        rowy = (int)(k % A.rows);
        tile = ((k / A.rows) << 3) + (blockIdx.x & 7);
    }
    if (tile >= A.ntiles) return;
    if (A.stop != nullptr && *A.stop != 0) return;
    const int64_t g0 = tile * S4_TG;
    S4_STAT(A.stats, 96 + 0, 1);
    static_assert(!(TAIL && LIST), "the row-walking launch takes its candidates in bin order");
    int nch[4], total = 0;
    const int64_t st4 = LIST ? (tile / (S4_STG / S4_TG)) * 4 : 0;
#pragma unroll
    for (int k = 0; k < 4; k++) { nch[k] = ((LIST ? A.stcount[st4 + k] : *A.k[k].nk) + 63) >> 6; total += nch[k]; }
    bool ran = false, weird = false;
    unsigned live = 0;
    const uint64_t *staged_en = nullptr;
    const double *staged_pts = nullptr;
    (void)staged_en;
    (void)staged_pts;
#define RH_S4_BODY(K)                                                                                                  \
    {                                                                                                                  \
        const int slo = max(lo, base) - base, shi = min(hi, base + nch[K]) - base;                                     \
        if (slo < shi) {                                                                                               \
            if (ran) __syncthreads();           \
            if (!ran || A.k[K].en != staged_en || A.k[K].pts != staged_pts) {    \
                s4_stage(sh, A.k[K].pts, A.k[K].stride, s, A.k[K].en, g0 * 64, A.k[K].gb32, A.k[K].gm32, A.ngroups);   \
                staged_en = A.k[K].en;                                                                                 \
                staged_pts = A.k[K].pts;                                                                               \
                S4_STAT(A.stats, 96 + 1, 1);                                                                           \
            } else { S4_STAT(A.stats, 96 + 2, 1); if (threadIdx.x == 0) { sh.npairs = 0; sh.next_batch = 0; } }      \
            __syncthreads();                                                                                           \
            live = 0;                                                                                                  \
            for (int g = 0; g < S4_TG; g++) live |= sh.len[g] != 0 ? (1u << g) : 0u;                                   \
            live = __builtin_amdgcn_readfirstlane(live);                                                               \
            { int ww = 0; for (int g = 0; g < S4_TG; g++) ww |= sh.weirdw[g]; weird = __builtin_amdgcn_readfirstlane(ww) != 0; }  \
            if (live != 0) score4_segment<K, R, MASK, F32, LIST>(sh, A.k[K], LIST ? A.stcount + (st4 + K) : A.k[K].nk, LIST ? A.stlist + (st4 + K) * A.stcap : nullptr, A.bstride, slo, shi, A.k[K].pts, A.k[K].stride, g0, live, weird, counts, dbg, A.masks, A.occ, A.mstride, A.stats); \
            else S4_STAT(A.stats, 96 + 3, 1);                                                                         \
            ran = true;                                                                                                \
        }                                                                                                              \
        base += nch[K];                                                                                                \
    }
    if (!TAIL) {
        const int lo = rowy * R, hi = min(total, lo + R);
        if (lo >= hi) return;
        int base = 0;
        RH_S4_BODY(RH_CONE)
        RH_S4_BODY(RH_CYLINDER)
        RH_S4_BODY(RH_SPHERE)
        RH_S4_BODY(RH_PLANE)
    } else {
        for (int lo = (A.row0 + (int)blockIdx.y) * R; lo < total; lo += (int)gridDim.y * R) {
            const int hi = min(total, lo + R);
            int base = 0;
            RH_S4_BODY(RH_CONE)
            RH_S4_BODY(RH_CYLINDER)
            RH_S4_BODY(RH_SPHERE)
            RH_S4_BODY(RH_PLANE)
        }
    }
#undef RH_S4_BODY
}

struct StCullArgs {
    const float *box[4];
    const int32_t *nk[4];
    int64_t bstride, stcap;
    const float *st32, *st32_plane;
    const uint32_t *stm32;
    uint16_t *stlist;
    int32_t *stcount;
};

template <int KIND>
static __device__ __forceinline__ void st_cull_kind(const StCullArgs &A, const int64_t st)
{
    constexpr int Q = 4;
    __shared__ int32_t wsum[2][Q * 4];
    const int tid = threadIdx.x, lane = tid & 63, wv = tid >> 6;
    const int nk = *A.nk[KIND];
    int32_t *cnt = A.stcount + st * 4 + KIND;
    if (nk <= 0) { if (tid == 0) *cnt = 0; return; }
    rh_box32 G;
    {
        const float *b = (KIND == RH_PLANE ? A.st32_plane : A.st32) + st * 8;
        G.cx = b[0]; G.cy = b[1]; G.cz = b[2]; G.hx = b[3]; G.hy = b[4]; G.hz = b[5]; G.hr = b[6];
    }
    rh_u32x4 GM = { 0xffffffffu, 0xffffffffu, 0xffffffffu, 0u };
    if (KIND == RH_PLANE && A.stm32 != nullptr) GM = ((const rh_u32x4 *)A.stm32)[st];
    uint16_t *__restrict__ list = A.stlist + (st * 4 + KIND) * A.stcap;
    constexpr int NB = S4Fields<KIND>::NBOX;
    const float *__restrict__ box = A.box[KIND];
    int base = 0, it = 0;
    for (int j0 = 0; j0 < nk; j0 += Q * 256, it++) {
        float B[Q][RH_BOX_FIELDS];
#pragma unroll
        for (int q = 0; q < Q; q++) {
            const int cand = j0 + q * 256 + tid, cl = cand < nk ? cand : 0;
#pragma unroll
            for (int f = 0; f < NB; f++) B[q][f] = box[(int64_t)f * A.bstride + cl];
        }
        uint64_t m[Q];
        bool keep[Q];
#pragma unroll
        for (int q = 0; q < Q; q++) {
            keep[q] = j0 + q * 256 + tid < nk && !box_skip32<KIND>(B[q], G);
            if (KIND == RH_PLANE) keep[q] = keep[q] && nsig_meet(B[q], GM);
            m[q] = WB(keep[q]);
            if (lane == 0) wsum[it & 1][q * 4 + wv] = __popcll(m[q]);
        }
        __syncthreads();
        int run = base;
#pragma unroll
        for (int q = 0; q < Q; q++) {
            int off = run;
#pragma unroll
            for (int w = 0; w < 4; w++) { const int v = wsum[it & 1][q * 4 + w]; off += w < wv ? v : 0; run += v; }
            if (keep[q]) list[off + __builtin_amdgcn_mbcnt_hi((uint32_t)(m[q] >> 32), __builtin_amdgcn_mbcnt_lo((uint32_t)m[q], 0))] = (uint16_t)(j0 + q * 256 + tid);
        }
        base = run;
    }
    if (tid == 0) *cnt = base;
}

__global__ void __launch_bounds__(256)
st_cull_kernel(const StCullArgs A)
{
    const int64_t st = blockIdx.x;
    switch (blockIdx.y) {
    case RH_PLANE: st_cull_kind<RH_PLANE>(A, st); break;
    case RH_SPHERE: st_cull_kind<RH_SPHERE>(A, st); break;
    case RH_CYLINDER: st_cull_kind<RH_CYLINDER>(A, st); break;
    default: st_cull_kind<RH_CONE>(A, st); break;
    }
}

}

#ifndef RH_PLANE_ORDER_MIN_TILES
#define RH_PLANE_ORDER_MIN_TILES 256
#endif
bool rhk_plane_order_wanted(const rh_cloud *c)
{
    if (c->pl_sub == nullptr) return false;
    const int64_t opt = rh_opt_int(c, RH_OPT_PLANE_ORDER, 0);
    return opt == 1 || (opt == 0 && (c->ngroups + S4_TG - 1) / S4_TG >= RH_PLANE_ORDER_MIN_TILES);
}

static inline int64_t stlist_bytes(const rh_cloud *c, int64_t cap) { return (int64_t)sizeof(uint16_t) * c->nst * 4 * cap; }
static int ensure_stlists(rh_cloud *c, rh_batch_ws &w, int64_t cap)
{
    if (w.d_stlist != nullptr && cap <= w.stlist_cap && w.stlist_nst == c->nst) return RH_OK;
    const int64_t ncap = std::max<int64_t>(cap, 1024);
    w.stlist_cap = 0;
    RH_TRY(w.d_stcount.grow(c->stream, c->nst * 4));
    RH_TRY(w.d_stlist.grow(c->stream, c->nst * 4 * ncap));
    w.stlist_cap = ncap;
    w.stlist_nst = c->nst;
    return RH_OK;
}

int rhk_score4_all(rh_cloud *c, rh_batch_ws &w, const rh_score_job &job, int32_t *launch_info)
{
    const rh_bins &B = job.bins;
    const int32_t nk_total_bound = job.bound;
    int32_t *const d_counts = job.d_counts;
    uint64_t *const d_masks_int = job.d_masks_int;
    const bool open_count = job.open_count;
    const bool f32cloud = c->f32;
    const bool on_subset = job.points.pts == nullptr;
    const rh_s4_points PS = on_subset ? rh_s4_points{ c->sub, c->s_pad, c->s, c->ngroups, c->gb32 } : job.points;
    const int64_t ntiles = (PS.ngroups + S4_TG - 1) / S4_TG;
    const int nchunks = cdiv4(nk_total_bound, 64) + 3;
    if (ntiles == 0 || nk_total_bound <= 0) return RH_OK;
    if (B.cls[0] == nullptr || B.box[0] == nullptr || !rh_score_v4_enabled(c) || PS.gb32 == nullptr || (d_masks_int != nullptr && !w.masks4)) {
        rh_set_error("internal: the culled score kernel without its records (classifier, culling, group boxes, mask lists)");
        return RH_E_INTERNAL;
    }
    const int dbg = (int)rh_opt_int(c, RH_OPT_G2_DBG, 0);
    const bool nsig_on = on_subset && c->gm32 != nullptr && rh_opt_int(c, RH_OPT_NSIG, 0) != 2;
    S4AllArgs A;
    for (int k = 0; k < 4; k++)
        A.k[k] = { (const rh_cls *)B.cls[k], B.box[k], B.prep[k], B.orig[k], job.nk[k], job.en[k], job.eps[k], job.cosa[k],
                   PS.pts, PS.stride, PS.gb32, nsig_on ? (const uint32_t *)c->gm32 : nullptr };
    const bool plane_on = on_subset && d_masks_int == nullptr && dbg == 0 && rhk_plane_order_wanted(c) &&
                          (job.en[RH_PLANE] == nullptr || job.en[RH_PLANE] == c->sub_enabled.get());
    if (plane_on) {
        S4KindArgs &P = A.k[RH_PLANE];
        P.pts = c->pl_sub;
        P.gb32 = c->pl_gb32;
        if (nsig_on) P.gm32 = c->pl_gm32;
        if (P.en != nullptr) P.en = c->pl_enabled;
    }
    A.stop = job.stop;
    A.ntiles = ntiles;
    A.bstride = job.bstride;
    A.ngroups = PS.ngroups;
    A.masks = d_masks_int;
    A.occ = d_masks_int ? w.d_occ : nullptr;
    A.mstride = d_masks_int ? w.mstride4 : 0;
    A.stats = nullptr;
#ifdef RH_DIAG
    A.stats = c->s4_stats;
#endif
    A.stlist = nullptr; A.stcount = nullptr; A.stcap = 0;
    const int64_t st_opt = rh_opt_int(c, RH_OPT_ST_CULL, 0);
    bool use_lists = !open_count && on_subset && dbg == 0 && c->st32 != nullptr && c->nst >= 2 && nk_total_bound <= 16384 && st_opt != 2;
    if (use_lists && st_opt == 0)
        use_lists = nk_total_bound >= 1024 && ntiles >= (rh_opt_int(c, RH_OPT_BATCHES_IN_FLIGHT, 1) > 1 ? 1000 : 3000);
    const int64_t lcap = std::max<int64_t>(((int64_t)nk_total_bound + 63) / 64 * 64, 1024);
    if (use_lists) {
        const int64_t mb = rh_opt_int(c, RH_OPT_ST_LIST_MB, 0);
        const int64_t need = stlist_bytes(c, lcap);
        if (need > ((mb > 0 ? mb : 512) << 20) || (w.stlist_nomem > 0 && need >= w.stlist_nomem)) use_lists = false;
    }
    if (use_lists) {
        const int rc = ensure_stlists(c, w, lcap);
        if (rc == RH_E_NOMEM) {
            (void)hipGetLastError();
            rh_set_error("%s", "");
            w.stlist_nomem = stlist_bytes(c, lcap);
            use_lists = false;
        } else if (rc != RH_OK) return rc;
    }
    if (use_lists) {
        StCullArgs SA;
        for (int k = 0; k < 4; k++) { SA.box[k] = B.box[k]; SA.nk[k] = job.nk[k]; }
        SA.bstride = job.bstride; SA.stcap = w.stlist_cap; SA.st32 = c->st32; SA.st32_plane = plane_on ? c->pl_st32 : c->st32;
        SA.stm32 = nsig_on && c->stm32 != nullptr ? (const uint32_t *)(plane_on ? c->pl_stm32 : c->stm32) : nullptr; SA.stlist = w.d_stlist; SA.stcount = w.d_stcount;
        hipLaunchKernelGGL(st_cull_kernel, dim3((unsigned)c->nst, 4), dim3(256), 0, c->stream, SA);
        A.stlist = w.d_stlist; A.stcount = w.d_stcount; A.stcap = w.stlist_cap;
        if (job.ev_listed != nullptr) RH_HIP(hipEventRecord(job.ev_listed, c->stream));
    }
    const int env_r = (int)rh_opt_int(c, RH_OPT_S4_ROWS, 0);
    int R;
    if (env_r == 4 || env_r == 8 || ((env_r == 1 || env_r == 2 || env_r == 12 || env_r == 16) && !open_count)) R = env_r;
    else if (open_count) R = ntiles * ((nchunks + 7) / 8) < 3000 ? 4 : 8;
    else if (ntiles * ((nchunks + 15) / 16) >= 16384) R = 16;
    else if (ntiles * ((nchunks + 11) / 12) >= 3000) R = use_lists ? 16 : 12;
    else if (ntiles * ((nchunks + 3) / 4) >= 4000) R = 4;
    else R = 2;
    int64_t rows = (nchunks + R - 1) / R;
    if (!open_count && launch_info != nullptr) { launch_info[0] = R; launch_info[1] = use_lists ? 1 : 0; launch_info[2] = (int32_t)rows; launch_info[3] = (int32_t)ntiles; }
    if (rows > 65535) { rh_set_error("batch of %d candidates is too large for one launch", nk_total_bound); return RH_E_INVALID; }
    const bool pad8 = ntiles >= 1024;
    dim3 grid((unsigned)(pad8 ? ((ntiles + 7) / 8) * 8 : ntiles), (unsigned)rows);
    const unsigned tiles_x = grid.x;
    A.row0 = 0;
    A.rows = 0;
#ifndef RH_S4_XROW_MAX
#define RH_S4_XROW_MAX 4096
#endif
    if (rows > 1 && ((ntiles + 7) / 8) * 8 * rows <= RH_S4_XROW_MAX) {
        A.rows = (int)rows;
        grid = dim3((unsigned)(((ntiles + 7) / 8) * 8 * rows), 1);
    }
    const int loop_max = open_count ? 32 : 0;
    auto launch_tail = [&](unsigned ny) {
        const dim3 gt(tiles_x, ny);
        if (f32cloud) {
            if (R == 4) hipLaunchKernelGGL((score4_kernel<4, false, true, true>), gt, dim3(64 * S4_W), 0, c->stream, PS.s, A, d_counts, dbg);
            else hipLaunchKernelGGL((score4_kernel<8, false, true, true>), gt, dim3(64 * S4_W), 0, c->stream, PS.s, A, d_counts, dbg);
        } else {
            if (R == 4) hipLaunchKernelGGL((score4_kernel<4, false, false, true>), gt, dim3(64 * S4_W), 0, c->stream, PS.s, A, d_counts, dbg);
            else hipLaunchKernelGGL((score4_kernel<8, false, false, true>), gt, dim3(64 * S4_W), 0, c->stream, PS.s, A, d_counts, dbg);
        }
    };
    if (loop_max > 0 && d_masks_int == nullptr && nchunks <= loop_max) {
        launch_tail(1);
        RH_HIP(hipGetLastError());
        return RH_OK;
    }
#define RH_S4_LAUNCH(RR, MM, FF)                                                                                                              \
    do {                                                                                                                                      \
// ... 69 lines not shown
```

### ransac.jl_amd/csrc/score4_device.h

```cpp
#pragma once

#include "rh_internal.h"

namespace rh4 {

constexpr double RH_CLS_U = 5.9604644775390625e-08;
constexpr double RH_CLS_SAFETY = 2.0;
constexpr double RH_CLS_BIG = 1048576.0;

struct rh_cls {
    float f[16];
};
constexpr int RH_CLS_FLAG = 15;

constexpr int RH_BOX_FIELDS = 11;
constexpr float RH_CONE_ALPHA = (float)((RH_CLS_SAFETY * 49.0 + 64.0) * RH_CLS_U);

__host__ __device__ inline bool cls_fin(double v) { return v - v == 0.0; }

__host__ __device__ inline float cls_dn(double v) { return (float)(v - fabs(v) * (2.0 * RH_CLS_U) - 1e-37); }
__host__ __device__ inline float cls_up(double v) { return (float)(v + fabs(v) * (2.0 * RH_CLS_U) + 1e-37); }

__host__ __device__ inline double cls_slack64(const rh_prep &P, double M) { return 1e-9 * ((1.0 + M) + P.f[11]); }

constexpr int RH_NSIG_CELLS = 96;


__host__ __device__ inline int nsig_cell(double x, double y, double z)
{
    const double ax = fabs(x), ay = fabs(y), az = fabs(z);
    double m, a, b;
    int axis;
    if (ax >= ay && ax >= az) { axis = 0; m = x; a = y; b = z; }
    else if (ay >= az) { axis = 1; m = y; a = z; b = x; }
    else { axis = 2; m = z; a = x; b = y; }
    const double h = 0.5 * fabs(m);
    const int i = (a >= -h ? 1 : 0) + (a >= 0.0 ? 1 : 0) + (a >= h ? 1 : 0);
    const int j = (b >= -h ? 1 : 0) + (b >= 0.0 ? 1 : 0) + (b >= h ? 1 : 0);
    return (axis * 2 + (m < 0.0 ? 1 : 0)) * 16 + i * 4 + j;
}

__host__ __device__ inline void nsig_point_bits(double nx, double ny, double nz, uint32_t w[3])
{
    w[0] = w[1] = w[2] = 0u;
    const double ax = fabs(nx), ay = fabs(ny), az = fabs(nz);
    if (ax == __builtin_inf() || ay == __builtin_inf() || az == __builtin_inf()) { w[0] = w[1] = w[2] = 0xffffffffu; return; }
    if (!(nx == nx) || !(ny == ny) || !(nz == nz) || (ax == 0.0 && ay == 0.0 && az == 0.0)) return;
    const int k = nsig_cell(nx, ny, nz);
    w[k >> 5] = 1u << (k & 31);
}

__host__ __device__ inline void nsig_cand_mask(double nx, double ny, double nz, double thr, double L, uint32_t m[3])
{
    static constexpr double tab[16][5] = {
        { 0.68599434057003528, -0.51449575542752646, -0.51449575542752646, 0.97182484440108552, 0.23570420404567663 },
        { 0.78446454055273618, -0.58834840541455213, -0.19611613513818404, 0.96076836812840516, 0.27735201964990502 },
        { 0.78446454055273618, -0.58834840541455213, 0.19611613513818404, 0.96076836812840516, 0.27735201964990502 },
        { 0.68599434057003528, -0.51449575542752646, 0.51449575542752646, 0.97182484440108552, 0.23570420404567663 },
        { 0.78446454055273618, -0.19611613513818404, -0.58834840541455213, 0.96076836812840516, 0.27735201964990502 },
        { 0.94280904158206347, -0.23570226039551587, -0.23570226039551587, 0.94280837491351122, 0.33333521895074958 },
        { 0.94280904158206347, -0.23570226039551587, 0.23570226039551587, 0.94280837491351122, 0.33333521895074958 },
        { 0.78446454055273618, -0.19611613513818404, 0.58834840541455213, 0.96076836812840516, 0.27735201964990502 },
        { 0.78446454055273618, 0.19611613513818404, -0.58834840541455213, 0.96076836812840516, 0.27735201964990502 },
        { 0.94280904158206347, 0.23570226039551587, -0.23570226039551587, 0.94280837491351122, 0.33333521895074958 },
        { 0.94280904158206347, 0.23570226039551587, 0.23570226039551587, 0.94280837491351122, 0.33333521895074958 },
        { 0.78446454055273618, 0.19611613513818404, 0.58834840541455213, 0.96076836812840516, 0.27735201964990502 },
        { 0.68599434057003528, 0.51449575542752646, -0.51449575542752646, 0.97182484440108552, 0.23570420404567663 },
        { 0.78446454055273618, 0.58834840541455213, -0.19611613513818404, 0.96076836812840516, 0.27735201964990502 },
        { 0.78446454055273618, 0.58834840541455213, 0.19611613513818404, 0.96076836812840516, 0.27735201964990502 },
        { 0.68599434057003528, 0.51449575542752646, 0.51449575542752646, 0.97182484440108552, 0.23570420404567663 },
    };
    m[0] = m[1] = m[2] = 0xffffffffu;
    const double nn = sqrt((nx * nx + ny * ny) + nz * nz);
    if (!(thr > 0.0) || !(L > 0.0) || !(nn > 0.0) || !cls_fin(thr) || !cls_fin(L) || !cls_fin(nn)) return;
    double T = thr / (L * nn) * (1.0 - 1e-9);
    if (!(T > 0.0)) return;
    if (T > 1.0) T = 1.0;
    const double Sn = sqrt(fmax(0.0, 1.0 - T * T));
    const double ux = nx / nn, uy = ny / nn, uz = nz / nn;
    const double fm[3] = { ux, uy, uz }, fa[3] = { uy, uz, ux }, fb[3] = { uz, ux, uy };
    uint32_t w0 = 0u, w1 = 0u, w2 = 0u;
#pragma unroll
    for (int axis = 0; axis < 3; axis++)
#pragma unroll
        for (int neg = 0; neg < 2; neg++) {
            uint32_t bits = 0u;
            for (int r = 0; r < 16; r++) {
                const double c = ((neg ? -tab[r][0] : tab[r][0]) * fm[axis] + tab[r][1] * fa[axis]) + tab[r][2] * fb[axis];
                bits |= c >= T * tab[r][3] - Sn * tab[r][4] ? (1u << r) : 0u;
            }
            const int f = axis * 2 + neg;
            if (f < 2) w0 |= bits << (16 * (f & 1));
            else if (f < 4) w1 |= bits << (16 * (f & 1));
            else w2 |= bits << (16 * (f & 1));
        }
    m[0] = w0; m[1] = w1; m[2] = w2;
}


__host__ __device__ inline void cls_make(const rh_prep &P, int kind, double eps, double cosa, double M, double Nm, rh_cls &o,
                                         float *box, int64_t bstride, double *dbg4 = nullptr, bool f32cloud = false, double Ln = 0.0)
{
    const double u = RH_CLS_U, S = f32cloud ? 3.0 * RH_CLS_SAFETY : RH_CLS_SAFETY;
    const float fnan = __builtin_nanf("");
    for (int i = 0; i < 16; i++) o.f[i] = 0.0f;
    float bx[RH_BOX_FIELDS];
    for (int i = 0; i < RH_BOX_FIELDS; i++) bx[i] = fnan;
    bool ok = cls_fin(eps) && cls_fin(cosa) && cls_fin(M) && cls_fin(Nm) && M <= RH_CLS_BIG && Nm <= RH_CLS_BIG && fabs(eps) <= RH_CLS_BIG;
    const double slack64 = cls_slack64(P, M);
    if (kind == RH_PLANE) {
        bool fin = true;
        for (int i = 0; i < 9; i++) fin = fin && cls_fin(P.f[i]) && fabs(P.f[i]) <= RH_CLS_BIG;
        ok = ok && fin;
        const double n1 = (fabs(P.f[3]) + fabs(P.f[4])) + fabs(P.f[5]);
        const double z1 = (fabs(P.f[6]) + fabs(P.f[7])) + fabs(P.f[8]);
        const double zp = (P.f[6] * P.f[0] + P.f[7] * P.f[1]) + P.f[8] * P.f[2];
        const double mN = S * u * (5.05 * (n1 * Nm) + 4.1 * (fabs(cosa) + 1e-3)) + 1e-30;
        const double zabs = (fabs(P.f[6] * P.f[0]) + fabs(P.f[7] * P.f[1])) + fabs(P.f[8] * P.f[2]);
        const double mRef = f32cloud ? RH_CLS_SAFETY * u * 6.2 * (z1 * M + zabs) : 0.0;
        const double mD = S * u * (6.1 * (z1 * M + fabs(zp)) + 4.0 * fabs(eps)) + mRef + 1e-30;
        ok = ok && cls_fin(mN) && cls_fin(mD) && cls_fin(zp) && mN < 1e30 && mD < 1e30;
        if (ok) {
            const double wN = 2.0 * mN, wD = 2.0 * mD;
            const double iN = 1.0 / wN, iD = 1.0 / wD;
            const double cNhi = cosa + 0.5 * wN, eDlo = eps - 0.5 * wD;
            ok = cosa - 0.5 * wN > 0.0;
            o.f[0] = (float)(-P.f[3] * iN); o.f[1] = (float)(-P.f[4] * iN); o.f[2] = (float)(-P.f[5] * iN);
            o.f[3] = (float)(cNhi * iN);
            o.f[4] = (float)(P.f[6] * iD); o.f[5] = (float)(P.f[7] * iD); o.f[6] = (float)(P.f[8] * iD);
            o.f[7] = (float)(-zp * iD);
            o.f[8] = (float)(eDlo * iD);
            if (dbg4 != nullptr) { dbg4[0] = cNhi; dbg4[1] = wN; dbg4[2] = eDlo; dbg4[3] = wD; }
            for (int i = 0; i < 9; i++) ok = ok && fabs((double)o.f[i]) < 1e30;
        }
        uint32_t cm[3] = { 0xffffffffu, 0xffffffffu, 0xffffffffu };
        if (ok) {
            const double Lb = 1.7320508075688774 * Nm * (1.0 + 1e-12);
            nsig_cand_mask(P.f[3], P.f[4], P.f[5], cosa - mN, (Ln > 0.0 && Ln < Lb ? Ln * (1.0 + 1e-12) : Lb), cm);
        }
        bx[5] = __builtin_bit_cast(float, cm[0]); bx[6] = __builtin_bit_cast(float, cm[1]); bx[7] = __builtin_bit_cast(float, cm[2]);
        if (fin && cls_fin(zp) && cls_fin(eps) && cls_fin(M)) {
            const double sB = S * 10.1 * u * (z1 * M + fabs(zp)) + mRef + slack64;
            bx[0] = (float)P.f[6]; bx[1] = (float)P.f[7]; bx[2] = (float)P.f[8];
            bx[3] = (float)(-zp);
            bx[4] = cls_up(eps + sB);
        }
    } else if (kind == RH_SPHERE || kind == RH_CYLINDER) {
        const bool sph = kind == RH_SPHERE;
        bool fin = true;
        for (int i = 0; i < 7; i++) fin = fin && ((sph && i >= 4) || (cls_fin(P.f[i]) && fabs(P.f[i]) <= RH_CLS_BIG));
        ok = ok && fin;
        const double R = sph ? P.f[3] : P.f[6], sgn = sph ? P.f[4] : P.f[7];
        const double c0 = sph ? P.f[0] : P.f[3], c1 = sph ? P.f[1] : P.f[4], c2 = sph ? P.f[2] : P.f[5];
        const double T = M + fmax(fabs(c0), fmax(fabs(c1), fabs(c2)));
        double e, lipk = 1.0;
        double a1 = 0.0, ai = 0.0;
        bool axis_ok = true;
        if (sph) {
            e = 2.01 * u * T;
        } else {
            a1 = (fabs(P.f[0]) + fabs(P.f[1])) + fabs(P.f[2]);
            ai = fmax(fabs(P.f[0]), fmax(fabs(P.f[1]), fabs(P.f[2])));
            axis_ok = ai <= 16.0;
            ok = ok && axis_ok;
            e = u * T * (3.01 + 8.04 * ai * a1);
            lipk = fmax(1.0, fabs(P.f[9] - 1.0));
        }
        const double s3 = 1.7320508075688774;
        const double mD = S * (s3 * e + 7.0 * u * (fabs(R) + fabs(eps))) + 1e-30;
        const double nrmax = R + eps + 3.0 * mD, nrmin = R - eps - 3.0 * mD;
        const double nq = nrmax + s3 * e;
        const double K = R * R + eps * eps, H = 2.0 * R * eps, ca2 = cosa * cosa;
        const double dn2 = 2.0 * nrmax * s3 * e + 3.0 * e * e + 4.0 * u * nq * nq + 6.0 * u * K;
        const double m2 = S * dn2 + 1e-30;
        const double ds = 3.0 * Nm * e + 5.0 * u * Nm * s3 * nq;
        const double mv = S * (2.0 * (fabs(cosa) * nrmax + ds) * ds + ds * ds + ca2 * dn2 + 8.0 * u * ca2 * nq * nq) + 1e-30;
        const double n2min = (R - eps) * (R - eps) - 2.0 * m2;
        ok = ok && cls_fin(m2) && cls_fin(mv) && (sgn == 1.0 || sgn == -1.0) && m2 < 1e30 && mv < 1e30;
        ok = ok && eps >= 0.0 && cosa > 0.0 && nrmin > 0.0 && n2min > 0.0 && ca2 * n2min > 1.001 * mv;
        if (sph) { o.f[0] = (float)P.f[0]; o.f[1] = (float)P.f[1]; o.f[2] = (float)P.f[2]; }
        else { o.f[0] = (float)P.f[0]; o.f[1] = (float)P.f[1]; o.f[2] = (float)P.f[2]; o.f[3] = (float)P.f[3]; o.f[4] = (float)P.f[4]; o.f[5] = (float)P.f[5]; }
        if (ok) {
            const double W2 = 2.0 * m2, Wv = 2.0 * mv;
            const double i2 = 1.0 / W2, iv = 1.0 / Wv;
            const float s0 = (float)K, s1 = (float)i2, s2 = (float)(-(H - m2) * i2), s3f = (float)(-sgn * iv), s4 = (float)(ca2 * iv);
            if (dbg4 != nullptr) { dbg4[0] = m2; dbg4[1] = W2; dbg4[2] = mv; dbg4[3] = Wv; }
            if (sph) { o.f[3] = s0; o.f[4] = s1; o.f[5] = s2; o.f[6] = s3f; o.f[7] = s4; }
            else { o.f[6] = s0; o.f[7] = s1; o.f[8] = s2; o.f[9] = s3f; o.f[10] = s4; }
            const double big = 1.329227995784916e36;
            const double n2max = 3.1 * T * T * ((1.0 + ai * a1) * (1.0 + ai * a1)), qn2max = 3.0 * Nm * Nm * n2max;
            ok = ok && fabs((double)s0) < 1e30 && fabs((double)s1) < 1e30 && fabs((double)s2) < 1e30 && fabs((double)s3f) < 1e30 && fabs((double)s4) < 1e30;
            ok = ok && (n2max + K) * i2 < big && qn2max * iv < big && n2max * ca2 * iv < big;
        }
        if (fin && axis_ok && (sph || a1 > 0.0) && cls_fin(eps) && cls_fin(M)) {
            const double sB = S * (s3 * e + 4.0 * u * (fabs(R) + fabs(eps)) + 4.0 * u * lipk * s3 * M) + slack64;
            const double A = (R + eps) + sB, B = (R - eps) - sB;
            if (cls_fin(A) && cls_fin(B)) {
                if (sph) {
                    bx[0] = (float)P.f[0]; bx[1] = (float)P.f[1]; bx[2] = (float)P.f[2];
                    bx[3] = A > 0.0 ? cls_up(A * A * (1.0 + 16.0 * u)) : 0.0f;
                    bx[4] = B > 0.0 ? cls_dn(B * B * (1.0 - 16.0 * u)) : -1.0f;
                } else {
                    for (int i = 0; i < 6; i++) bx[i] = (float)P.f[i];
                    bx[6] = cls_up(A);
                    bx[7] = cls_dn(B);
                    bx[8] = cls_up(lipk);
                    const double As = A + S * 3.01 * u * (2.0 + 8.0 * ai * a1) * M;
                    const double r2max = 3.1 * T * T * ((1.0 + ai * a1) * (1.0 + ai * a1));
                    if (cls_fin(As) && r2max < 1e18) bx[9] = As > 0.0 ? cls_up(As * As * (1.0 + 16.0 * u)) : 0.0f;
                }
            }
        }
    } else {
        for (int i = 0; i < 8; i++) ok = ok && cls_fin(P.f[i]) && fabs(P.f[i]) <= RH_CLS_BIG;
        const double ax = P.f[3], ay = P.f[4], az = P.f[5], c = P.f[6], sn = P.f[7], sgn = P.f[8];
        const double an = sqrt((ax * ax + ay * ay) + az * az), cs = sqrt(c * c + sn * sn);
        ok = ok && (an > 1e-300) && cls_fin(an) && (cs > 1e-300) && cls_fin(cs) && (sgn == 1.0 || sgn == -1.0);
        const bool band_ok = ok && (c > 1e-6 * cs);
        const double ia = ok ? 1.0 / an : 0.0;
        const double T = M + fmax(fabs(P.f[0]), fmax(fabs(P.f[1]), fabs(P.f[2])));
        const double kk = band_ok ? -sn / c : 0.0;
// ... 249 lines not shown
```

### ransac.jl_amd/csrc/score4_diag.hip

```cpp
#ifdef RH_DIAG
#include <stdio.h>
#include <stdlib.h>

#include <algorithm>
#include <vector>

#include "rh_internal.h"
#include "ransac_hip_diag.h"
#include "score_device.h"
#include "score4_device.h"
#include "score4_shared.h"
#include "wave_keys.h"

namespace {

using namespace rhdev;
using namespace rh4;

struct S4AuditCand { rh_prep P; rh_cls C; double cNhi, wN, eDlo, wD, cosa, eps; int kind, usable; };

__global__ void __launch_bounds__(256)
cls_audit_kernel(const double *__restrict__ pts, int64_t stride, int64_t s, const S4AuditCand *__restrict__ cands, int ncand,
                 unsigned long long *__restrict__ out)
{
// ... 5 lines not shown
    bool counted = false;
    if (i < s && Q.usable) {
        const double x = pts[i], y = pts[stride + i], z = pts[2 * stride + i];
        const double nx = pts[3 * stride + i], ny = pts[4 * stride + i], nz = pts[5 * stride + i];
        const rh_prep &P = Q.P;
        float a32, b32;
        double a64, b64;
        if (Q.kind == RH_PLANE) {
            cls_plane_ab(Q.C, (float)x, (float)y, (float)z, (float)nx, (float)ny, (float)nz, a32, b32);
            const double dn = (P.f[3] * nx + P.f[4] * ny) + P.f[5] * nz;
            const double d = (P.f[6] * (x - P.f[0]) + P.f[7] * (y - P.f[1])) + P.f[8] * (z - P.f[2]);
            a64 = (Q.cNhi - dn) / Q.wN;
            b64 = (fabs(d) - Q.eDlo) / Q.wD;
            ea = fabs((double)a32 - a64);
            eb = fabs((double)b32 - b64);
            counted = true;
        } else if (Q.kind == RH_SPHERE || Q.kind == RH_CYLINDER) {
            double qx, qy, qz, R, sgn;
            if (Q.kind == RH_SPHERE) {
                cls_round_ab<RH_SPHERE>(Q.C, (float)x, (float)y, (float)z, (float)nx, (float)ny, (float)nz, a32, b32);
                qx = x - P.f[0]; qy = y - P.f[1]; qz = z - P.f[2]; R = P.f[3]; sgn = P.f[4];
            } else {
                cls_round_ab<RH_CYLINDER>(Q.C, (float)x, (float)y, (float)z, (float)nx, (float)ny, (float)nz, a32, b32);
                const double tx = x - P.f[3], ty = y - P.f[4], tz = z - P.f[5];
                const double sd = (P.f[0] * tx + P.f[1] * ty) + P.f[2] * tz;
                qx = (x - P.f[0] * sd) - P.f[3]; qy = (y - P.f[1] * sd) - P.f[4]; qz = (z - P.f[2] * sd) - P.f[5];
                R = P.f[6]; sgn = P.f[7];
            }
            const double m2 = Q.cNhi, W2 = Q.wN, mv = Q.eDlo, Wv = Q.wD;
            const double n2 = (qx * qx + qy * qy) + qz * qz;
            const double qn = (qx * nx + qy * ny) + qz * nz;
            a64 = (fabs(n2 - (R * R + Q.eps * Q.eps)) - (2.0 * R * Q.eps - m2)) / W2;
            b64 = (mv + (Q.cosa * Q.cosa * n2 - sgn * qn * fabs(qn))) / Wv;
            if (a64 < 2.0) { ea = fabs((double)a32 - a64); eb = fabs((double)b32 - b64); }
            counted = true;
        } else if (Q.kind == RH_CONE) {
            bool near_axis;
            cls_cone_ab(Q.C, (float)x, (float)y, (float)z, (float)nx, (float)ny, (float)nz, a32, b32, near_axis);
            if (!near_axis) {
                double dist, dt;
                cone_frame(P, x, y, z, nx, ny, nz, dist, dt);
                const double an = sqrt((P.f[3] * P.f[3] + P.f[4] * P.f[4]) + P.f[5] * P.f[5]);
                const double wx = x - P.f[0], wy = y - P.f[1], wz = z - P.f[2];
                const double h = ((P.f[3] * wx + P.f[4] * wy) + P.f[5] * wz) / an;
                const double qx = wx - h * (P.f[3] / an), qy = wy - h * (P.f[4] / an), qz = wz - h * (P.f[5] / an);
                const double rho = sqrt((qx * qx + qy * qy) + qz * qz);
                a64 = (fabs(dist) - Q.eDlo) / Q.wD;
                b64 = 0.5 - rho * (P.f[8] * dt - Q.cosa) / Q.wN;
                ea = fabs((double)a32 - a64);
                eb = fabs((double)b32 - b64);
                counted = true;
            }
        }
        if (!(ea == ea)) ea = 1e30;
        if (!(eb == eb)) eb = 1e30;
    }
    __shared__ unsigned long long sa[4], sb[4];
    __shared__ int sc[4];
    unsigned long long ua = __builtin_bit_cast(unsigned long long, ea), ub = __builtin_bit_cast(unsigned long long, eb);
    int cnt = counted ? 1 : 0;
    for (int off = 32; off > 0; off >>= 1) {
        const unsigned long long va = __shfl_down(ua, off), vb = __shfl_down(ub, off);
        ua = va > ua ? va : ua;
        ub = vb > ub ? vb : ub;
        cnt += __shfl_down(cnt, off);
    }
    if ((threadIdx.x & 63) == 0) { sa[threadIdx.x >> 6] = ua; sb[threadIdx.x >> 6] = ub; sc[threadIdx.x >> 6] = cnt; }
    __syncthreads();
    if (threadIdx.x == 0 && Q.kind >= 0 && Q.kind < 4) {
        unsigned long long ma = 0, mb = 0;
        int n = 0;
        for (int w = 0; w < 4; w++) { ma = sa[w] > ma ? sa[w] : ma; mb = sb[w] > mb ? sb[w] : mb; n += sc[w]; }
        atomicMax(&out[Q.kind * 2], ma);
        atomicMax(&out[Q.kind * 2 + 1], mb);
        atomicAdd(&out[8 + Q.kind], (unsigned long long)n);
    }
}

struct S4SoundCand { rh_prep P; rh_prepf Pf; rh_cls C; float box[RH_BOX_FIELDS]; int kind; int pad; };
struct S4SoundArgs { double eps[4], cosa[4]; int f32; };

template <int KIND>
static __device__ __forceinline__ void sound_one(const S4SoundCand &Q, const S4SoundArgs &A, double x, double y, double z, double nx, double ny,
                                                 double nz, const uint64_t valid, const rh_box32 &G, const rh_box32 &GS, const rh_box32 &GT, const rh_u32x4 gm, const rh_u32x4 sm, const int lane, unsigned long long *__restrict__ out)
{
    const double eps = A.eps[KIND], cosa = A.cosa[KIND];
    uint64_t ex;
    if (A.f32) ex = test_point<KIND>(Q.Pf, (float)x, (float)y, (float)z, (float)nx, (float)ny, (float)nz, eps, cosa);
    else ex = test_point<KIND>(Q.P, x, y, z, nx, ny, nz, eps, cosa);
    ex &= valid;
    const bool skip = box_skip32<KIND>(Q.box, G);
    const bool stskip = box_skip32<KIND>(Q.box, GS);
    const bool tlskip = box_skip32<KIND>(Q.box, GT);
    const bool exact_only = is_nan_bits(Q.C.f[RH_CLS_FLAG]);
    const float fx = (float)x, fy = (float)y, fz = (float)z, fnx = (float)nx, fny = (float)ny, fnz = (float)nz;
    float t, t0;
    if (KIND == RH_PLANE) { t = cls_plane_u(Q.C, fx, fy, fz, fnx, fny, fnz); t0 = cls_plane_u(Q.C, 0.f, 0.f, 0.f, 0.f, 0.f, 0.f); }
    else if (KIND == RH_CONE) { t = cls_cone_u(Q.C, fx, fy, fz, fnx, fny, fnz); t0 = 0.5f; }
    else { t = cls_round_u<KIND == RH_SPHERE ? RH_SPHERE : RH_CYLINDER>(Q.C, fx, fy, fz, fnx, fny, fnz);
           t0 = cls_round_u<KIND == RH_SPHERE ? RH_SPHERE : RH_CYLINDER>(Q.C, 0.f, 0.f, 0.f, 0.f, 0.f, 0.f); }
    const float sum = (fabsf(fx) + fabsf(fy)) + (fabsf(fz) + fabsf(fnx)) + (fabsf(fny) + fabsf(fnz));
    const bool weird = WB(!(sum < __builtin_inff()) && ((valid >> lane) & 1ULL)) != 0;
    const bool decided = !exact_only && !weird;
    const uint64_t sin_ = WB(decided && cls_sure(t)) & valid;
    const uint64_t amb = (WB(!decided || (KIND == RH_CONE ? (!cls_sure(t) && cls_sure(t - 1.0f)) : cls_undecided(t)))) & valid;
    const uint64_t sout = valid & ~sin_ & ~amb;
    float du, dn;
    bool near_axis = false;
    if (KIND == RH_PLANE) cls_plane_ab(Q.C, fx, fy, fz, fnx, fny, fnz, dn, du);
    else if (KIND == RH_CONE) cls_cone_ab(Q.C, fx, fy, fz, fnx, fny, fnz, du, dn, near_axis);
    else cls_round_ab<KIND == RH_SPHERE ? RH_SPHERE : RH_CYLINDER>(Q.C, fx, fy, fz, fnx, fny, fnz, du, dn);
    const uint64_t band = WB(!decided || near_axis || !(du > 1.0f)) & valid;
    if (lane == 0) {
        if (band != 0) atomicAdd(&out[40 + KIND], 1ULL);
        if (ex != 0) atomicAdd(&out[44 + KIND], 1ULL);
        if (stskip) atomicAdd(&out[48 + KIND], 1ULL);
        if (stskip && ex != 0) atomicAdd(&out[52 + KIND], 1ULL);
        if (tlskip) atomicAdd(&out[56 + KIND], 1ULL);
        if (tlskip && ex != 0) atomicAdd(&out[60 + KIND], 1ULL);
        if (KIND == RH_PLANE) {
            const bool gskip = !nsig_meet(Q.box, gm), sskip = !nsig_meet(Q.box, sm);
            if (gskip) atomicAdd(&out[64], 1ULL);
            if (gskip && ex != 0) atomicAdd(&out[65], 1ULL);
            if (sskip) atomicAdd(&out[66], 1ULL);
            if (sskip && ex != 0) atomicAdd(&out[67], 1ULL);
        }
        unsigned long long *o = out + KIND * 10;
        atomicAdd(&o[0], 1ULL);
        if (skip) atomicAdd(&o[1], 1ULL);
        if (skip && ex != 0) atomicAdd(&o[2], 1ULL);
        atomicAdd(&o[3], (unsigned long long)__popcll(valid));
        if (sin_) atomicAdd(&o[4], (unsigned long long)__popcll(sin_));
        if (sout) atomicAdd(&o[5], (unsigned long long)__popcll(sout));
        if (sin_ & ~ex) atomicAdd(&o[6], (unsigned long long)__popcll(sin_ & ~ex));
        if (sout & ex) atomicAdd(&o[7], (unsigned long long)__popcll(sout & ex));
        if (ex) atomicAdd(&o[8], (unsigned long long)__popcll(ex));
        if (blockIdx.x == 0 && !exact_only && cls_sure(t0)) atomicAdd(&o[9], 1ULL);
    }
}

__global__ void __launch_bounds__(64)
cls_sound_kernel(const double *__restrict__ pts, int64_t stride, int64_t s, const float *__restrict__ gb32, const float *__restrict__ st32, const float *__restrict__ tile32, const uint32_t *__restrict__ gm32, const uint32_t *__restrict__ stm32, const S4SoundCand *__restrict__ cands,
                 int ncand, const S4SoundArgs A, const int kinds, unsigned long long *__restrict__ out)
{
    const int lane = threadIdx.x;
    const int64_t g = blockIdx.x;
    const int64_t i = g * 64 + lane;
    const uint64_t valid = valid_mask(g * 64, s);
    const bool on = (valid >> lane) & 1ULL;
    const double x = on ? pts[i] : 0.0, y = on ? pts[stride + i] : 0.0, z = on ? pts[2 * stride + i] : 0.0;
    const double nx = on ? pts[3 * stride + i] : 0.0, ny = on ? pts[4 * stride + i] : 0.0, nz = on ? pts[5 * stride + i] : 0.0;
    rh_box32 G;
    G.cx = gb32[g * 8 + 0]; G.cy = gb32[g * 8 + 1]; G.cz = gb32[g * 8 + 2]; G.hx = gb32[g * 8 + 3];
    G.hy = gb32[g * 8 + 4]; G.hz = gb32[g * 8 + 5]; G.hr = gb32[g * 8 + 6];
    rh_box32 GS;
    {
        const float *b = st32 + (g / S4_STG) * 8;
        GS.cx = b[0]; GS.cy = b[1]; GS.cz = b[2]; GS.hx = b[3]; GS.hy = b[4]; GS.hz = b[5]; GS.hr = b[6];
    }
    rh_box32 GT;
    {
        const float *b = tile32 + (g / S4_TG) * 8;
        GT.cx = b[0]; GT.cy = b[1]; GT.cz = b[2]; GT.hx = b[3]; GT.hy = b[4]; GT.hz = b[5]; GT.hr = b[6];
    }
    const rh_u32x4 gm = ((const rh_u32x4 *)gm32)[g], sm = ((const rh_u32x4 *)stm32)[g / S4_STG];
    for (int c = blockIdx.y; c < ncand; c += gridDim.y) {
        const S4SoundCand &Q = cands[c];
        if (Q.kind < 0 || Q.kind > 3 || !((kinds >> Q.kind) & 1)) continue;
        switch (Q.kind) {
        case RH_PLANE: sound_one<RH_PLANE>(Q, A, x, y, z, nx, ny, nz, valid, G, GS, GT, gm, sm, lane, out); break;
        case RH_SPHERE: sound_one<RH_SPHERE>(Q, A, x, y, z, nx, ny, nz, valid, G, GS, GT, gm, sm, lane, out); break;
        case RH_CYLINDER: sound_one<RH_CYLINDER>(Q, A, x, y, z, nx, ny, nz, valid, G, GS, GT, gm, sm, lane, out); break;
        case RH_CONE: sound_one<RH_CONE>(Q, A, x, y, z, nx, ny, nz, valid, G, GS, GT, gm, sm, lane, out); break;
        default: break;
        }
    }
}

__global__ void __launch_bounds__(256)
cls_cone_dbg_kernel(const rh_cls C, const float *__restrict__ pts, int64_t n, float *__restrict__ ua, float *__restrict__ ub,
                    uint8_t *__restrict__ near_out)
{
    const int64_t i = (int64_t)blockIdx.x * blockDim.x + threadIdx.x;
    if (i >= n) return;
    float a, b;
    bool near_axis;
    cls_cone_ab(C, pts[i], pts[n + i], pts[2 * n + i], pts[3 * n + i], pts[4 * n + i], pts[5 * n + i], a, b, near_axis);
    ua[i] = a;
    ub[i] = b;
    near_out[i] = near_axis ? 1 : 0;
}

struct Probe {
    rh_prep P;
    rh_cls C;
    float box[RH_BOX_FIELDS];
    double d4[4];
};

int probe_make(const char *who, const char *only, int kinds, const rh_shape *shape, const rh_params *p, double M, double Nm, double Ln, int f32,
               Probe &Q, float *rec_out = nullptr, float *fields_out = nullptr, double *dbg4_out = nullptr)
{
    const int kind = shape->kind;
    if (kind < 0 || kind > 3 || !((kinds >> kind) & 1)) { rh_set_error("%s: %s only", who, only); return RH_E_INVALID; }
    rh_prep_host(*shape, &Q.P);
    for (int k = 0; k < 4; k++) Q.d4[k] = 0;
    cls_make(Q.P, kind, p->eps[kind], p->cos_alpha[kind], M, Nm, Q.C, Q.box, 1, Q.d4, f32 != 0, Ln);
    if (rec_out != nullptr)
        for (int k = 0; k < 16; k++) rec_out[k] = Q.C.f[k];
    if (fields_out != nullptr)
        for (int k = 0; k < RH_BOX_FIELDS; k++) fields_out[k] = Q.box[k];
    if (dbg4_out != nullptr)
        for (int k = 0; k < 4; k++) dbg4_out[k] = Q.d4[k];
    return RH_OK;
}

rh_box32 probe_box(const double *b)
{
    float o[8];
    box_to_f32(b, b + 3, o);
    rh_box32 G;
    G.cx = o[0]; G.cy = o[1]; G.cz = o[2]; G.hx = o[3]; G.hy = o[4]; G.hz = o[5]; G.hr = o[6];
    return G;
}

void probe_point(const double *xyz, const double *nrm, int64_t i, float q[6])
{
    for (int k = 0; k < 3; k++) { q[k] = (float)xyz[3 * i + k]; q[3 + k] = (float)nrm[3 * i + k]; }
}

}

extern "C" int rh_dbg_cls_audit(rh_cloud *c, const rh_shape *shapes, int32_t b, const rh_params *p, double *out)
{
    if (c == nullptr || out == nullptr || p == nullptr || b < 0 || (b > 0 && shapes == nullptr)) { rh_set_error("rh_dbg_cls_audit: bad arguments"); return RH_E_INVALID; }
    for (int i = 0; i < 12; i++) out[i] = 0.0;
    if (b == 0 || c->s == 0) return RH_OK;
    RH_HIP(hipSetDevice(c->device));
    std::vector<S4AuditCand> h((size_t)b);
    for (int32_t i = 0; i < b; i++) {
        S4AuditCand &Q = h[(size_t)i];
        Q.kind = shapes[i].kind;
        Q.usable = 0;
        if (Q.kind < 0 || Q.kind > 3) continue;
        rh_prep_host(shapes[i], &Q.P);
        double d4[4] = { 0, 0, 0, 0 };
        cls_make(Q.P, Q.kind, p->eps[Q.kind], p->cos_alpha[Q.kind], c->coord_mag, c->nrm_mag, Q.C, nullptr, 0, d4, c->f32);
        Q.cNhi = d4[0]; Q.wN = d4[1]; Q.eDlo = d4[2]; Q.wD = d4[3]; Q.cosa = p->cos_alpha[Q.kind]; Q.eps = p->eps[Q.kind];
        Q.usable = !(Q.C.f[RH_CLS_FLAG] != Q.C.f[RH_CLS_FLAG]) && Q.wN > 0 && Q.wD > 0;
    }
    rh_dev<S4AuditCand> d_c;
    rh_dev<unsigned long long> d_o;
    RH_TRY(d_c.alloc(b));
    RH_TRY(d_o.alloc(12));
    RH_HIP(hipMemcpyAsync(d_c, h.data(), sizeof(S4AuditCand) * (size_t)b, hipMemcpyHostToDevice, c->stream));
    RH_HIP(hipMemsetAsync(d_o, 0, sizeof(unsigned long long) * 12, c->stream));
    for (int32_t c0 = 0; c0 < b; c0 += 32768) {
        const int32_t nb = std::min<int32_t>(32768, b - c0);
        hipLaunchKernelGGL(cls_audit_kernel, dim3((unsigned)cdiv4(c->s, 256), (unsigned)nb), dim3(256), 0, c->stream, c->sub, c->s_pad,
                           c->s, d_c + c0, nb, d_o);
    }
    unsigned long long ho[12];
    RH_HIP(hipMemcpyAsync(ho, d_o, sizeof ho, hipMemcpyDeviceToHost, c->stream));
    RH_HIP(hipStreamSynchronize(c->stream));
    for (int i = 0; i < 8; i++) out[i] = __builtin_bit_cast(double, ho[i]);
    for (int i = 8; i < 12; i++) out[i] = (double)ho[i];
    return RH_OK;
}

static int cls_soundness_run(rh_cloud *c, const rh_shape *shapes, int32_t b, const rh_params *p, uint64_t *out, const int first, const int nout)
{
    if (c == nullptr || out == nullptr || p == nullptr || b < 0 || (b > 0 && shapes == nullptr)) { rh_set_error("rh_dbg_cls_soundness: bad arguments"); return RH_E_INVALID; }
    for (int i = 0; i < nout; i++) out[i] = 0;
    if (b == 0 || c->s == 0 || c->ngroups == 0 || c->gb32 == nullptr || c->st32 == nullptr || c->tile32 == nullptr || c->gm32 == nullptr || c->stm32 == nullptr) return RH_OK;
    RH_HIP(hipSetDevice(c->device));
    std::vector<S4SoundCand> h((size_t)b);
    for (int32_t i = 0; i < b; i++) {
        S4SoundCand &Q = h[(size_t)i];
        Q.kind = shapes[i].kind;
        Q.pad = 0;
        if (Q.kind < 0 || Q.kind > 3) { Q.kind = -1; continue; }
        rh_prep_host(shapes[i], &Q.P);
        Q.Pf = prepf_of_kind(Q.P, Q.kind);
        cls_make(Q.P, Q.kind, p->eps[Q.kind], p->cos_alpha[Q.kind], c->coord_mag, c->nrm_mag, Q.C, Q.box, 1, nullptr, c->f32, c->nrm_len);
    }
    S4SoundArgs A;
    for (int k = 0; k < 4; k++) { A.eps[k] = p->eps[k]; A.cosa[k] = p->cos_alpha[k]; }
    A.f32 = c->f32 ? 1 : 0;
    rh_dev<S4SoundCand> d_c;
    rh_dev<unsigned long long> d_o;
    RH_TRY(d_c.alloc(b));
    RH_TRY(d_o.alloc(72));
    RH_HIP(hipMemcpyAsync(d_c, h.data(), sizeof(S4SoundCand) * (size_t)b, hipMemcpyHostToDevice, c->stream));
    RH_HIP(hipMemsetAsync(d_o, 0, sizeof(unsigned long long) * 72, c->stream));
    const bool pl = rhk_plane_order_wanted(c);
    const dim3 grid((unsigned)c->ngroups, (unsigned)std::min<int32_t>(b, 64));
    hipLaunchKernelGGL(cls_sound_kernel, grid, dim3(64), 0, c->stream, c->sub, c->s_pad, c->s, c->gb32, c->st32, c->tile32, c->gm32, c->stm32, d_c, b, A,
                       pl ? 0xe : 0xf, d_o);
    rh_dev<double> pl_gb;
    rh_dev<float> pl_tile32;
    if (pl) {
        RH_TRY(pl_gb.alloc(7 * c->ng_pad));
        RH_TRY(pl_tile32.alloc(8 * std::max<int64_t>(1, c->ntile)));
        RH_HIP(hipMemsetAsync(pl_gb, 0, sizeof(double) * 7 * (size_t)c->ng_pad, c->stream));
        RH_TRY(rhk_group_bounds_of(c, c->pl_sub, c->s_pad, c->s, c->ngroups, pl_gb, c->ng_pad));
        rhk_runs32_of(c, pl_gb, S4_TG, c->ntile, pl_tile32);
        hipLaunchKernelGGL(cls_sound_kernel, grid, dim3(64), 0, c->stream, c->pl_sub, c->s_pad, c->s, c->pl_gb32, c->pl_st32, pl_tile32, c->pl_gm32, c->pl_stm32, d_c,
                           b, A, 0x1, d_o);
    }
    RH_HIP(hipGetLastError());
    unsigned long long ho[72];
    RH_HIP(hipMemcpyAsync(ho, d_o, sizeof ho, hipMemcpyDeviceToHost, c->stream));
    RH_HIP(hipStreamSynchronize(c->stream));
    for (int i = 0; i < nout; i++) out[i] = (uint64_t)ho[first + i];
    return RH_OK;
}

extern "C" int rh_dbg_cls_soundness(rh_cloud *c, const rh_shape *shapes, int32_t b, const rh_params *p, uint64_t *out)
{
    return cls_soundness_run(c, shapes, b, p, out, 0, 56);
}

extern "C" int rh_dbg_cls_soundness_tiles(rh_cloud *c, const rh_shape *shapes, int32_t b, const rh_params *p, uint64_t *out)
{
    return cls_soundness_run(c, shapes, b, p, out, 56, 8);
}

extern "C" int rh_dbg_cls_soundness_nsig(rh_cloud *c, const rh_shape *shapes, int32_t b, const rh_params *p, uint64_t *out)
{
    return cls_soundness_run(c, shapes, b, p, out, 64, 4);
}

extern "C" int rh_dbg_nsig(const rh_shape *shape, const rh_params *p, double M, double Nm, double Ln, int f32, uint32_t *mask_out,
                           const double *dirs, int64_t ndirs, int32_t *cells_out)
{
    if (p == nullptr || ndirs < 0 || (ndirs > 0 && (dirs == nullptr || cells_out == nullptr)) || (shape != nullptr && mask_out == nullptr)) {
        rh_set_error("rh_dbg_nsig: bad arguments");
        return RH_E_INVALID;
    }
    if (shape != nullptr) {
        Probe Q;
        RH_TRY(probe_make("rh_dbg_nsig", "planes", 1 << RH_PLANE, shape, p, M, Nm, Ln, f32, Q));
        for (int k = 0; k < 3; k++) mask_out[k] = __builtin_bit_cast(uint32_t, Q.box[5 + k]);
    }
    for (int64_t i = 0; i < ndirs; i++) {
        uint32_t w[3];
        nsig_point_bits(dirs[3 * i], dirs[3 * i + 1], dirs[3 * i + 2], w);
        if ((w[0] & w[1] & w[2]) == 0xffffffffu) cells_out[i] = -2;
        else if ((w[0] | w[1] | w[2]) == 0u) cells_out[i] = -1;
        else cells_out[i] = nsig_cell(dirs[3 * i], dirs[3 * i + 1], dirs[3 * i + 2]);
    }
    return RH_OK;
}

extern "C" int rh_dbg_group_boxes(rh_cloud *c, double *out, int64_t cap, int64_t *ngroups_out)
{
    if (c == nullptr || ngroups_out == nullptr || cap < 0) { rh_set_error("rh_dbg_group_boxes: bad arguments"); return RH_E_INVALID; }
    *ngroups_out = c->gb == nullptr ? 0 : c->ngroups;
    if (out == nullptr || cap < *ngroups_out || *ngroups_out == 0) return RH_OK;
    RH_HIP(hipSetDevice(c->device));
    std::vector<double> h((size_t)c->ngroups * 6);
    const double *gb = c->gb;
    for (int k = 0; k < 6; k++)
        RH_HIP(hipMemcpyAsync(h.data() + (size_t)k * c->ngroups, gb + (int64_t)k * c->ng_pad, sizeof(double) * (size_t)c->ngroups, hipMemcpyDeviceToHost, c->stream));
    RH_HIP(hipStreamSynchronize(c->stream));
    for (int64_t g = 0; g < c->ngroups; g++)
        for (int k = 0; k < 6; k++) out[6 * g + k] = h[(size_t)k * c->ngroups + g];
    return RH_OK;
}

extern "C" int rh_dbg_cylbox(const rh_shape *shape, const rh_params *p, double M, double Nm, int f32, const double *boxes, int64_t n,
                             uint8_t *skip_out, uint8_t *ball_out, float *fields_out)
{
    if (shape == nullptr || p == nullptr || n < 0 || (n > 0 && (boxes == nullptr || skip_out == nullptr || ball_out == nullptr))) {
        rh_set_error("rh_dbg_cylbox: bad arguments");
        return RH_E_INVALID;
    }
    Probe Q;
    RH_TRY(probe_make("rh_dbg_cylbox", "cylinders", 1 << RH_CYLINDER, shape, p, M, Nm, 0.0, f32, Q, nullptr, fields_out));
    for (int64_t i = 0; i < n; i++) {
        const rh_box32 G = probe_box(boxes + 6 * i);
        skip_out[i] = cyl_box_skip32<true>(Q.box, G) ? 1 : 0;
        ball_out[i] = cyl_box_skip32<false>(Q.box, G) ? 1 : 0;
    }
    return RH_OK;
}

extern "C" int rh_dbg_cls_round(const rh_shape *shape, const rh_params *p, double M, double Nm, int f32, int64_t n, const double *xyz,
                                const double *nrm, float *ua_out, float *ub_out, float *rec_out, double *dbg4_out)
{
    if (shape == nullptr || p == nullptr || n < 0 || (n > 0 && (xyz == nullptr || nrm == nullptr || ua_out == nullptr || ub_out == nullptr))) {
        rh_set_error("rh_dbg_cls_round: bad arguments");
        return RH_E_INVALID;
    }
    Probe Q;
    RH_TRY(probe_make("rh_dbg_cls_round", "spheres and cylinders", (1 << RH_SPHERE) | (1 << RH_CYLINDER), shape, p, M, Nm, 0.0, f32, Q, rec_out, nullptr, dbg4_out));
    for (int64_t i = 0; i < n; i++) {
        float q[6];
        probe_point(xyz, nrm, i, q);
        if (shape->kind == RH_SPHERE) cls_round_ab<RH_SPHERE>(Q.C, q[0], q[1], q[2], q[3], q[4], q[5], ua_out[i], ub_out[i]);
        else cls_round_ab<RH_CYLINDER>(Q.C, q[0], q[1], q[2], q[3], q[4], q[5], ua_out[i], ub_out[i]);
    }
    return RH_OK;
}

extern "C" int rh_dbg_books2(const float *u2, int64_t nseq, int32_t *sure_count_out, uint64_t *sure_word_out, uint64_t *und_word_out,
                             uint8_t *any_und_out)
{
    if (nseq < 0 || (nseq > 0 && (u2 == nullptr || sure_count_out == nullptr || sure_word_out == nullptr || und_word_out == nullptr || any_und_out == nullptr))) {
        rh_set_error("rh_dbg_books2: bad arguments");
        return RH_E_INVALID;
    }
    for (int64_t s = 0; s < nseq; s++) {
// ... 102 lines not shown
```

### ransac.jl_amd/csrc/score4_shared.h

```cpp
#pragma once

#include "rh_internal.h"
#include "score4_device.h"

namespace {

typedef float rh_f32x4 __attribute__((ext_vector_type(4)));
typedef float rh_f32x2 __attribute__((ext_vector_type(2)));
typedef unsigned long long rh_u64x2 __attribute__((ext_vector_type(2)));
typedef uint32_t rh_u32x4 __attribute__((ext_vector_type(4)));

constexpr int S4_TG = RH_G2_TG;
constexpr int S4_STG = RH_S4_STG;

static __device__ __forceinline__ bool is_nan_bits(float v)
{
    return (__builtin_bit_cast(uint32_t, v) & 0x7fffffffu) > 0x7f800000u;
}

template <int KIND> struct S4Fields { static constexpr int NBOX = KIND == RH_PLANE ? 8 : (KIND == RH_SPHERE ? 5 : (KIND == RH_CYLINDER ? 10 : 11)); };

static __device__ __forceinline__ bool nsig_meet(const float (&B)[rh4::RH_BOX_FIELDS], const rh_u32x4 gm)
{
    return (((__builtin_bit_cast(uint32_t, B[5]) & gm.x) | (__builtin_bit_cast(uint32_t, B[6]) & gm.y)) | (__builtin_bit_cast(uint32_t, B[7]) & gm.z)) != 0u;
}

inline int cdiv4(int64_t a, int64_t b) { return (int)((a + b - 1) / b); }

}
```

Before: 89.06 million candidates/s.

## Add per-group normal-cone bounds to cull plane candidates in scoring

```diff
diff --git a/include/ransac_hip_diag.h b/include/ransac_hip_diag.h
--- a/include/ransac_hip_diag.h
+++ b/include/ransac_hip_diag.h
@@ -13,6 +13,10 @@
 int rh_dbg_cls_soundness_nsig(rh_cloud *c, const rh_shape *shapes, int32_t b, const rh_params *p, uint64_t *out );
 int rh_dbg_nsig(const rh_shape *shape, const rh_params *p, double M, double Nm, double Ln, int f32, uint32_t *mask_out ,
                 const double *dirs, int64_t ndirs, int32_t *cells_out);
+int rh_dbg_cls_soundness_ncone(rh_cloud *c, const rh_shape *shapes, int32_t b, const rh_params *p, uint64_t *out );
+int rh_dbg_ncone(const double *normals, int32_t cnt, float *cone_out , const rh_shape *shapes, int32_t nshapes, const rh_params *p,
+                 double M, double Nm, double Ln, int f32, float *fields_out, int32_t *meet_out);
+int rh_dbg_ncones(rh_cloud *c, int which, float *out, int64_t cap, int64_t *ngroups_out);
 int rh_dbg_group_boxes(rh_cloud *c, double *out, int64_t cap, int64_t *ngroups_out);
 int rh_dbg_kd_shape(int64_t s, int aligned, int64_t *info_out , int64_t *nodes_out, int64_t node_cap, int64_t *splits_out,
                     int64_t split_cap, int64_t *leaves_out, int64_t leaf_cap);
diff --git a/ransac.jl_amd/_lib.py b/ransac.jl_amd/_lib.py
--- a/ransac.jl_amd/_lib.py
+++ b/ransac.jl_amd/_lib.py
@@ -306,6 +306,9 @@
     "rh_dbg_cls_soundness": (C.c_int, [_vp, _sp, C.c_int32, _pp, C.POINTER(C.c_uint64)]),
     "rh_dbg_cls_soundness_tiles": (C.c_int, [_vp, _sp, C.c_int32, _pp, C.POINTER(C.c_uint64)]),
     "rh_dbg_cls_soundness_nsig": (C.c_int, [_vp, _sp, C.c_int32, _pp, C.POINTER(C.c_uint64)]),
+    "rh_dbg_cls_soundness_ncone": (C.c_int, [_vp, _sp, C.c_int32, _pp, C.POINTER(C.c_uint64)]),
+    "rh_dbg_ncone": (C.c_int, [_dp, C.c_int32, C.POINTER(C.c_float), _sp, C.c_int32, _pp, C.c_double, C.c_double, C.c_double, C.c_int, C.POINTER(C.c_float), _i32p]),
+    "rh_dbg_ncones": (C.c_int, [_vp, C.c_int, C.POINTER(C.c_float), C.c_int64, C.POINTER(C.c_int64)]),
     "rh_dbg_nsig": (C.c_int, [_sp, _pp, C.c_double, C.c_double, C.c_double, C.c_int, C.POINTER(C.c_uint32), _dp, C.c_int64, _i32p]),
     "rh_dbg_group_boxes": (C.c_int, [_vp, _dp, C.c_int64, C.POINTER(C.c_int64)]),
     "rh_dbg_kd_shape": (C.c_int, [C.c_int64, C.c_int, _i64p, _i64p, C.c_int64, _i64p, C.c_int64, _i64p, C.c_int64]),
diff --git a/ransac.jl_amd/csrc/boxes32.hip b/ransac.jl_amd/csrc/boxes32.hip
--- a/ransac.jl_amd/csrc/boxes32.hip
+++ b/ransac.jl_amd/csrc/boxes32.hip
@@ -48,7 +48,8 @@
 }
 
 __global__ void __launch_bounds__(256)
-nsig_kernel(const double *__restrict__ pts, int64_t stride, int64_t s, int64_t ngroups, uint32_t *__restrict__ out, unsigned long long *__restrict__ maxlen)
+nsig_kernel(const double *__restrict__ pts, int64_t stride, int64_t s, int64_t ngroups, uint32_t *__restrict__ out, unsigned long long *__restrict__ maxlen,
+            float *__restrict__ cones)
 {
     __shared__ uint32_t m[4][4];
     const int lane = threadIdx.x & 63, wv = threadIdx.x >> 6;
@@ -57,8 +58,11 @@
     __syncthreads();
     const int64_t i = g * 64 + lane;
     double len = 0.0;
+    double d[3] = { 0.0, 0.0, 0.0 };
+    int dk = 0;
     if (g < ngroups && i < s) {
         const double nx = pts[3 * stride + i], ny = pts[4 * stride + i], nz = pts[5 * stride + i];
+        dk = ncone_dir(nx, ny, nz, d);
         uint32_t w[3];
         nsig_point_bits(nx, ny, nz, w);
         if (w[0] != 0u) atomicOr(&m[wv][0], w[0]);
@@ -70,6 +74,25 @@
     unsigned long long lb = __builtin_bit_cast(unsigned long long, len);
     for (int off = 32; off > 0; off >>= 1) { const unsigned long long v = __shfl_down(lb, off); lb = v > lb ? v : lb; }
     if (lane == 0 && lb != 0ULL) atomicMax(maxlen, lb);
+    if (cones != nullptr) {
+        double sx = d[0], sy = d[1], sz = d[2];
+        int cnt = dk == 1 ? 1 : 0, inf = dk == 2 ? 1 : 0;
+        for (int off = 32; off > 0; off >>= 1) {
+            sx += __shfl_down(sx, off); sy += __shfl_down(sy, off); sz += __shfl_down(sz, off);
+            cnt += __shfl_down(cnt, off); inf += __shfl_down(inf, off);
+        }
+        sx = __shfl(sx, 0); sy = __shfl(sy, 0); sz = __shfl(sz, 0); cnt = __shfl(cnt, 0); inf = __shfl(inf, 0);
+        double m[3];
+        const bool has_axis = ncone_axis(sx, sy, sz, cnt, m);
+        double cmin = dk == 1 ? (m[0] * d[0] + m[1] * d[1]) + m[2] * d[2] : __builtin_inf();
+        for (int off = 32; off > 0; off >>= 1) cmin = fmin(cmin, __shfl_down(cmin, off));
+        if (lane == 0 && g < ngroups) {
+            float o[4];
+            ncone_record(m, has_axis, cmin, cnt, inf != 0, o);
+#pragma unroll
+            for (int k = 0; k < 4; k++) cones[g * 4 + k] = o[k];
+        }
+    }
     __syncthreads();
     if (g < ngroups && lane < 4) out[g * 4 + lane] = m[wv][lane];
 }
@@ -91,6 +114,7 @@
     const double *gb;
     float *gb32, *st32, *tile32;
     uint32_t *gm32, *stm32;
+    float *gc32;
 };
 
 int twins32_build(rh_cloud *c, const Twins32 &T, double *nrm_len)
@@ -104,7 +128,7 @@
     rh_dev<unsigned long long> d_len;
     RH_TRY(d_len.alloc(1));
     RH_HIP(hipMemsetAsync(d_len, 0, sizeof(unsigned long long), c->stream));
-    hipLaunchKernelGGL(nsig_kernel, dim3(cdiv4(c->ngroups, 4)), dim3(256), 0, c->stream, T.pts, c->s_pad, c->s, c->ngroups, T.gm32, d_len);
+    hipLaunchKernelGGL(nsig_kernel, dim3(cdiv4(c->ngroups, 4)), dim3(256), 0, c->stream, T.pts, c->s_pad, c->s, c->ngroups, T.gm32, d_len, T.gc32);
     hipLaunchKernelGGL(nsig_st_kernel, dim3(cdiv4(c->nst, 64)), dim3(64), 0, c->stream, T.gm32, c->ngroups, S4_STG, c->nst, T.stm32);
     RH_HIP(hipGetLastError());
     unsigned long long h_len = 0;
@@ -129,7 +153,7 @@
 int rhk_gb32_build(rh_cloud *c)
 {
     if (c->ngroups == 0 || c->gb32 == nullptr) return RH_OK;
-    return twins32_build(c, { c->sub, c->gb, c->gb32, c->st32, c->tile32, c->gm32, c->stm32 }, &c->nrm_len);
+    return twins32_build(c, { c->sub, c->gb, c->gb32, c->st32, c->tile32, c->gm32, c->stm32, c->gc32 }, &c->nrm_len);
 }
 
 int rhk_plane_boxes(rh_cloud *c)
@@ -141,5 +165,5 @@
     RH_HIP(hipMemsetAsync(c->pl_gb32, 0, sizeof(float) * 8 * (size_t)c->ng_pad, c->stream));
     RH_HIP(hipMemsetAsync(c->pl_gm32, 0, sizeof(uint32_t) * 4 * (size_t)c->ng_pad, c->stream));
     RH_TRY(rhk_group_bounds_of(c, c->pl_sub, c->s_pad, c->s, c->ngroups, gb, c->ng_pad));
-    return twins32_build(c, { c->pl_sub, gb, c->pl_gb32, c->pl_st32, nullptr, c->pl_gm32, c->pl_stm32 }, nullptr);
+    return twins32_build(c, { c->pl_sub, gb, c->pl_gb32, c->pl_st32, nullptr, c->pl_gm32, c->pl_stm32, c->pl_gc32 }, nullptr);
 }
diff --git a/ransac.jl_amd/csrc/cloud.hip b/ransac.jl_amd/csrc/cloud.hip
--- a/ransac.jl_amd/csrc/cloud.hip
+++ b/ransac.jl_amd/csrc/cloud.hip
@@ -310,6 +310,7 @@
     c->ntile = (c->ngroups + RH_G2_TG - 1) / RH_G2_TG;
     CK(c->tile32.alloc(8 * std::max<int64_t>(1, c->ntile)));
     CK(c->gm32.alloc(4 * c->ng_pad));
+    CK(c->gc32.alloc(4 * c->ng_pad));
     CK(c->stm32.alloc(4 * std::max<int64_t>(1, c->nst)));
     CK(c->dis_gb.alloc(7 * c->ng_pad));
     CK(c->dis_gb32.alloc(8 * c->ng_pad));
diff --git a/ransac.jl_amd/csrc/kdorder.hip b/ransac.jl_amd/csrc/kdorder.hip
--- a/ransac.jl_amd/csrc/kdorder.hip
+++ b/ransac.jl_amd/csrc/kdorder.hip
@@ -440,6 +440,7 @@
     RH_TRY(c->pl_stm32.alloc(4 * c->nst));
     RH_TRY(c->pl_gb32.alloc(8 * c->ng_pad));
     RH_TRY(c->pl_gm32.alloc(4 * c->ng_pad));
+    RH_TRY(c->pl_gc32.alloc(4 * c->ng_pad));
     RH_TRY(c->pl_enabled.alloc(c->swords));
     RH_HIP(hipMemsetAsync(c->pl_sub, 0, sizeof(double) * 6 * (size_t)c->s_pad, c->stream));
     RH_HIP(hipMemsetAsync(c->pl_src, 0, sizeof(int32_t) * (size_t)c->s_pad, c->stream));
diff --git a/ransac.jl_amd/csrc/options.cpp b/ransac.jl_amd/csrc/options.cpp
--- a/ransac.jl_amd/csrc/options.cpp
+++ b/ransac.jl_amd/csrc/options.cpp
@@ -33,6 +33,7 @@
     RH_O(RH_OPT_NSIG, "nsig", "RH_NSIG", T_INT),
     RH_O(RH_OPT_PLANE_ORDER, "plane_order", "RH_PLANE_ORDER", T_INT),
     RH_O(RH_OPT_KD_ALIGN, "kd_align", "RH_KD_ALIGN", T_INT),
+    RH_O(RH_OPT_NCONE, "ncone", "RH_NCONE", T_INT),
 #ifdef RH_DIAG
     RH_O(RH_OPT_CREATE_PROF, "create_prof", "RH_CREATE_PROF", T_FLAG),
     RH_O(RH_OPT_AABB_HOST, "aabb_host", "RH_AABB_HOST", T_FLAG),
@@ -144,6 +145,7 @@
         case RH_OPT_BATCHES_IN_FLIGHT: ok = value >= 0 && value <= RH_MAX_IN_FLIGHT; break;
         case RH_OPT_ST_LIST_MB: ok = value >= 0 && value <= (1 << 20); break;
         case RH_OPT_NSIG: ok = value == 0 || value == 2; break;
+        case RH_OPT_NCONE: ok = value == 0 || value == 2; break;
         case RH_OPT_PLANE_ORDER: ok = value >= 0 && value <= 2; break;
         case RH_OPT_KD_ALIGN: ok = value >= 0 && value <= 2; break;
         default: break;
diff --git a/ransac.jl_amd/csrc/rh_internal.h b/ransac.jl_amd/csrc/rh_internal.h
--- a/ransac.jl_amd/csrc/rh_internal.h
+++ b/ransac.jl_amd/csrc/rh_internal.h
@@ -40,6 +40,7 @@
     RH_OPT_NSIG,
     RH_OPT_PLANE_ORDER,
     RH_OPT_KD_ALIGN,
+    RH_OPT_NCONE,
     RH_OPT_N_PRODUCT,
     RH_OPT_CREATE_PROF = RH_OPT_N_PRODUCT, RH_OPT_AABB_HOST, RH_OPT_SUB_ORDER, RH_OPT_KD_HOST, RH_OPT_NO_SPREAD, RH_OPT_OCT_CHAIN_W,
     RH_OPT_NO_MANAGED_STORE, RH_OPT_OCT_ONE_WINDOW, RH_OPT_OCT_WINDOW_ITERS, RH_OPT_NO_FUSED_SCORE, RH_OPT_NO_PIPELINE,
@@ -269,11 +270,13 @@
     int64_t ntile = 0;
     rh_dev<uint32_t> gm32;
     rh_dev<uint32_t> stm32;
+    rh_dev<float> gc32;
     double nrm_len = 0;
     rh_dev<double> pl_sub;
     rh_dev<int32_t> pl_src;
     rh_dev<float> pl_gb32;
     rh_dev<uint32_t> pl_gm32;
+    rh_dev<float> pl_gc32;
     rh_dev<float> pl_st32;
     rh_dev<uint32_t> pl_stm32;
     rh_dev<uint64_t> pl_enabled;
diff --git a/ransac.jl_amd/csrc/score4.hip b/ransac.jl_amd/csrc/score4.hip
--- a/ransac.jl_amd/csrc/score4.hip
+++ b/ransac.jl_amd/csrc/score4.hip
@@ -26,6 +26,7 @@
     uint64_t len[S4_TG];
     rh_f32x4 gbox[S4_TG][2];
     rh_u32x4 gmask[S4_TG];
+    rh_f32x4 gcone[S4_TG];
     uint16_t plist[R * 64 * S4_TG + 2];
     uint16_t ctab[LIST ? R * 64 : 2];
     int32_t cntb[S4_W][64];
@@ -52,6 +53,7 @@
     int row0;
     int rows;
     S4KindArgs k[4];
+    const float *gc32;
     int64_t ntiles, bstride, ngroups;
     uint64_t *masks;
     uint8_t *occ;
@@ -301,6 +303,7 @@
             G.cx = g0v.x; G.cy = g0v.y; G.cz = g0v.z; G.hx = g0v.w; G.hy = g1v.x; G.hz = g1v.y; G.hr = g1v.z;
             bool skip = box_skip32<KIND>(B[h & 1], G);
             if (KIND == RH_PLANE) skip |= !nsig_meet(B[h & 1], sh.gmask[g]);
+            if (KIND == RH_PLANE) skip |= !ncone_meet(B[h & 1], sh.gcone[g]);
             surv |= skip ? 0u : (1u << g);
         }
         if (dbg == 2) surv = (1u << S4_TG) - 1u;
@@ -340,7 +343,7 @@
 template <class SH>
 static __device__ __forceinline__ void s4_stage(SH &sh, const double *__restrict__ pts, int64_t stride, int64_t s,
                                                 const uint64_t *__restrict__ enabled_words, const int64_t p0, const float *__restrict__ gb32,
-                                                const uint32_t *__restrict__ gm32, const int64_t ngroups)
+                                                const uint32_t *__restrict__ gm32, const float *__restrict__ gc32, const int64_t ngroups)
 {
     static_assert(S4_TG % S4_W == 0, "every wave stages S4_TG / S4_W groups");
     const int tid = threadIdx.x, lane = tid & 63;
@@ -384,6 +387,12 @@
         if (gm32 != nullptr) m = ((const rh_u32x4 *)gm32)[g < ngroups ? g : ngroups - 1];
         sh.gmask[tid - 64] = m;
     }
+    if (tid >= 128 && tid < 128 + S4_TG) {
+        const int64_t g = p0 / 64 + (tid - 128);
+        rh_f32x4 cn = { 0.f, 0.f, 0.f, -__builtin_inff() };
+        if (gc32 != nullptr) cn = ((const rh_f32x4 *)gc32)[g < ngroups ? g : ngroups - 1];
+        sh.gcone[tid - 128] = cn;
+    }
 }
 
 template <int R, bool MASK, bool F32, bool TAIL = false, bool LIST = false>
@@ -428,7 +437,7 @@
         if (slo < shi) {                                                                                               \
             if (ran) __syncthreads();           \
             if (!ran || A.k[K].en != staged_en || A.k[K].pts != staged_pts) {    \
-                s4_stage(sh, A.k[K].pts, A.k[K].stride, s, A.k[K].en, g0 * 64, A.k[K].gb32, A.k[K].gm32, A.ngroups);   \
+                s4_stage(sh, A.k[K].pts, A.k[K].stride, s, A.k[K].en, g0 * 64, A.k[K].gb32, A.k[K].gm32, A.k[K].pts == A.k[RH_PLANE].pts ? A.gc32 : nullptr, A.ngroups);   \
                 staged_en = A.k[K].en;                                                                                 \
                 staged_pts = A.k[K].pts;                                                                               \
                 S4_STAT(A.stats, 96 + 1, 1);                                                                           \
@@ -492,7 +501,7 @@
     rh_u32x4 GM = { 0xffffffffu, 0xffffffffu, 0xffffffffu, 0u };
     if (KIND == RH_PLANE && A.stm32 != nullptr) GM = ((const rh_u32x4 *)A.stm32)[st];
     uint16_t *__restrict__ list = A.stlist + (st * 4 + KIND) * A.stcap;
-    constexpr int NB = S4Fields<KIND>::NBOX;
+    constexpr int NB = S4Fields<KIND>::NLIST;
     const float *__restrict__ box = A.box[KIND];
     int base = 0, it = 0;
     for (int j0 = 0; j0 < nk; j0 += Q * 256, it++) {
@@ -582,10 +591,12 @@
     }
     const int dbg = (int)rh_opt_int(c, RH_OPT_G2_DBG, 0);
     const bool nsig_on = on_subset && c->gm32 != nullptr && rh_opt_int(c, RH_OPT_NSIG, 0) != 2;
+    const bool ncone_on = nsig_on && c->gc32 != nullptr && rh_opt_int(c, RH_OPT_NCONE, 0) != 2;
     S4AllArgs A;
     for (int k = 0; k < 4; k++)
         A.k[k] = { (const rh_cls *)B.cls[k], B.box[k], B.prep[k], B.orig[k], job.nk[k], job.en[k], job.eps[k], job.cosa[k],
                    PS.pts, PS.stride, PS.gb32, nsig_on ? (const uint32_t *)c->gm32 : nullptr };
+    A.gc32 = ncone_on ? (const float *)c->gc32 : nullptr;
     const bool plane_on = on_subset && d_masks_int == nullptr && dbg == 0 && rhk_plane_order_wanted(c) &&
                           (job.en[RH_PLANE] == nullptr || job.en[RH_PLANE] == c->sub_enabled.get());
     if (plane_on) {
@@ -593,6 +604,7 @@
         P.pts = c->pl_sub;
         P.gb32 = c->pl_gb32;
         if (nsig_on) P.gm32 = c->pl_gm32;
+        if (ncone_on) A.gc32 = c->pl_gc32;
         if (P.en != nullptr) P.en = c->pl_enabled;
     }
     A.stop = job.stop;
diff --git a/ransac.jl_amd/csrc/score4_device.h b/ransac.jl_amd/csrc/score4_device.h
--- a/ransac.jl_amd/csrc/score4_device.h
+++ b/ransac.jl_amd/csrc/score4_device.h
@@ -97,6 +97,60 @@
     m[0] = w0; m[1] = w1; m[2] = w2;
 }
 
+constexpr double RH_NCONE_EPS = 2e-3;
+constexpr double RH_NCONE_COS_EPS = 0.99999800000066667;
+constexpr double RH_NCONE_SIN_EPS = 0.0019999986666669333;
+
+__host__ __device__ inline int ncone_dir(double nx, double ny, double nz, double d[3])
+{
+    d[0] = d[1] = d[2] = 0.0;
+    const double ax = fabs(nx), ay = fabs(ny), az = fabs(nz);
+    if (ax == __builtin_inf() || ay == __builtin_inf() || az == __builtin_inf()) return 2;
+    const double s = fmax(ax, fmax(ay, az));
+    if (!(nx == nx) || !(ny == ny) || !(nz == nz) || s == 0.0) return 0;
+    const double x = nx / s, y = ny / s, z = nz / s;
+    const double l = sqrt((x * x + y * y) + z * z);
+    d[0] = x / l; d[1] = y / l; d[2] = z / l;
+    return 1;
+}
+
+__host__ __device__ inline bool ncone_axis(double sx, double sy, double sz, int cnt, double m[3])
+{
+    const double l = sqrt((sx * sx + sy * sy) + sz * sz);
+    m[0] = m[1] = m[2] = 0.0;
+    if (cnt <= 0 || !(l > 1e-6 * (double)cnt)) return false;
+    m[0] = sx / l; m[1] = sy / l; m[2] = sz / l;
+    return true;
+}
+
+__host__ __device__ inline void ncone_record(const double m[3], bool has_axis, double cmin, int cnt, bool any_inf, float o[4])
+{
+    o[0] = o[1] = o[2] = 0.0f;
+    o[3] = -__builtin_inff();
+    if (any_inf) return;
+    if (cnt <= 0) { o[3] = __builtin_inff(); return; }
+    if (!has_axis || !(cmin == cmin)) return;
+    const double c = fmin(1.0, fmax(-1.0, cmin)), s = sqrt(fmax(0.0, 1.0 - c * c));
+    const double cg = c * RH_NCONE_COS_EPS - s * RH_NCONE_SIN_EPS, sg = s * RH_NCONE_COS_EPS + c * RH_NCONE_SIN_EPS;
+    if (!(cg > 0.0)) return;
+    const double is = 1.0 / sg;
+    o[0] = (float)(m[0] * is); o[1] = (float)(m[1] * is); o[2] = (float)(m[2] * is);
+    o[3] = (float)(cg * is);
+}
+
+__host__ __device__ inline void ncone_cand(double nx, double ny, double nz, double thr, double L, float o[2])
+{
+    o[0] = o[1] = __builtin_nanf("");
+    const double nn = sqrt((nx * nx + ny * ny) + nz * nz);
+    if (!(thr > 0.0) || !(L > 0.0) || !(nn > 0.0) || !cls_fin(thr) || !cls_fin(L) || !cls_fin(nn)) return;
+    double T = thr / (L * nn) * (1.0 - 1e-9);
+    if (!(T > 0.0)) return;
+    if (T > 1.0) T = 1.0;
+    const double Sn = sqrt(fmax(0.0, 1.0 - T * T));
+    o[0] = (float)T;
+    o[1] = (float)Sn;
+}
+
 
 __host__ __device__ inline void cls_make(const rh_prep &P, int kind, double eps, double cosa, double M, double Nm, rh_cls &o,
                                          float *box, int64_t bstride, double *dbg4 = nullptr, bool f32cloud = false, double Ln = 0.0)
@@ -136,7 +190,9 @@
         uint32_t cm[3] = { 0xffffffffu, 0xffffffffu, 0xffffffffu };
         if (ok) {
             const double Lb = 1.7320508075688774 * Nm * (1.0 + 1e-12);
-            nsig_cand_mask(P.f[3], P.f[4], P.f[5], cosa - mN, (Ln > 0.0 && Ln < Lb ? Ln * (1.0 + 1e-12) : Lb), cm);
+            const double Lu = Ln > 0.0 && Ln < Lb ? Ln * (1.0 + 1e-12) : Lb;
+            nsig_cand_mask(P.f[3], P.f[4], P.f[5], cosa - mN, Lu, cm);
+            ncone_cand(P.f[3], P.f[4], P.f[5], cosa - mN, Lu, bx + 8);
         }
         bx[5] = __builtin_bit_cast(float, cm[0]); bx[6] = __builtin_bit_cast(float, cm[1]); bx[7] = __builtin_bit_cast(float, cm[2]);
         if (fin && cls_fin(zp) && cls_fin(eps) && cls_fin(M)) {
diff --git a/ransac.jl_amd/csrc/score4_diag.hip b/ransac.jl_amd/csrc/score4_diag.hip
--- a/ransac.jl_amd/csrc/score4_diag.hip
+++ b/ransac.jl_amd/csrc/score4_diag.hip
@@ -111,7 +111,7 @@
 
 template <int KIND>
 static __device__ __forceinline__ void sound_one(const S4SoundCand &Q, const S4SoundArgs &A, double x, double y, double z, double nx, double ny,
-                                                 double nz, const uint64_t valid, const rh_box32 &G, const rh_box32 &GS, const rh_box32 &GT, const rh_u32x4 gm, const rh_u32x4 sm, const int lane, unsigned long long *__restrict__ out)
+                                                 double nz, const uint64_t valid, const rh_box32 &G, const rh_box32 &GS, const rh_box32 &GT, const rh_u32x4 gm, const rh_u32x4 sm, const rh_f32x4 gc, const int lane, unsigned long long *__restrict__ out)
 {
     const double eps = A.eps[KIND], cosa = A.cosa[KIND];
     uint64_t ex;
@@ -153,6 +153,11 @@
             if (gskip && ex != 0) atomicAdd(&out[65], 1ULL);
             if (sskip) atomicAdd(&out[66], 1ULL);
             if (sskip && ex != 0) atomicAdd(&out[67], 1ULL);
+            const bool cskip = !ncone_meet(Q.box, gc);
+            if (cskip) atomicAdd(&out[68], 1ULL);
+            if (cskip && ex != 0) atomicAdd(&out[69], 1ULL);
+            if (cskip && !skip && !gskip) atomicAdd(&out[70], 1ULL);
+            if (!cskip && !skip && !gskip) atomicAdd(&out[71], 1ULL);
         }
         unsigned long long *o = out + KIND * 10;
         atomicAdd(&o[0], 1ULL);
@@ -169,7 +174,7 @@
 }
 
 __global__ void __launch_bounds__(64)
-cls_sound_kernel(const double *__restrict__ pts, int64_t stride, int64_t s, const float *__restrict__ gb32, const float *__restrict__ st32, const float *__restrict__ tile32, const uint32_t *__restrict__ gm32, const uint32_t *__restrict__ stm32, const S4SoundCand *__restrict__ cands,
+cls_sound_kernel(const double *__restrict__ pts, int64_t stride, int64_t s, const float *__restrict__ gb32, const float *__restrict__ st32, const float *__restrict__ tile32, const uint32_t *__restrict__ gm32, const uint32_t *__restrict__ stm32, const float *__restrict__ gc32, const S4SoundCand *__restrict__ cands,
                  int ncand, const S4SoundArgs A, const int kinds, unsigned long long *__restrict__ out)
 {
     const int lane = threadIdx.x;
@@ -193,14 +198,16 @@
         GT.cx = b[0]; GT.cy = b[1]; GT.cz = b[2]; GT.hx = b[3]; GT.hy = b[4]; GT.hz = b[5]; GT.hr = b[6];
     }
     const rh_u32x4 gm = ((const rh_u32x4 *)gm32)[g], sm = ((const rh_u32x4 *)stm32)[g / S4_STG];
+    rh_f32x4 gc = { 0.f, 0.f, 0.f, -__builtin_inff() };
+    if (gc32 != nullptr) gc = ((const rh_f32x4 *)gc32)[g];
     for (int c = blockIdx.y; c < ncand; c += gridDim.y) {
         const S4SoundCand &Q = cands[c];
         if (Q.kind < 0 || Q.kind > 3 || !((kinds >> Q.kind) & 1)) continue;
         switch (Q.kind) {
-        case RH_PLANE: sound_one<RH_PLANE>(Q, A, x, y, z, nx, ny, nz, valid, G, GS, GT, gm, sm, lane, out); break;
-        case RH_SPHERE: sound_one<RH_SPHERE>(Q, A, x, y, z, nx, ny, nz, valid, G, GS, GT, gm, sm, lane, out); break;
-        case RH_CYLINDER: sound_one<RH_CYLINDER>(Q, A, x, y, z, nx, ny, nz, valid, G, GS, GT, gm, sm, lane, out); break;
-        case RH_CONE: sound_one<RH_CONE>(Q, A, x, y, z, nx, ny, nz, valid, G, GS, GT, gm, sm, lane, out); break;
+        case RH_PLANE: sound_one<RH_PLANE>(Q, A, x, y, z, nx, ny, nz, valid, G, GS, GT, gm, sm, gc, lane, out); break;
+        case RH_SPHERE: sound_one<RH_SPHERE>(Q, A, x, y, z, nx, ny, nz, valid, G, GS, GT, gm, sm, gc, lane, out); break;
+        case RH_CYLINDER: sound_one<RH_CYLINDER>(Q, A, x, y, z, nx, ny, nz, valid, G, GS, GT, gm, sm, gc, lane, out); break;
+        case RH_CONE: sound_one<RH_CONE>(Q, A, x, y, z, nx, ny, nz, valid, G, GS, GT, gm, sm, gc, lane, out); break;
         default: break;
         }
     }
@@ -324,7 +331,7 @@
     RH_HIP(hipMemsetAsync(d_o, 0, sizeof(unsigned long long) * 72, c->stream));
     const bool pl = rhk_plane_order_wanted(c);
     const dim3 grid((unsigned)c->ngroups, (unsigned)std::min<int32_t>(b, 64));
-    hipLaunchKernelGGL(cls_sound_kernel, grid, dim3(64), 0, c->stream, c->sub, c->s_pad, c->s, c->gb32, c->st32, c->tile32, c->gm32, c->stm32, d_c, b, A,
+    hipLaunchKernelGGL(cls_sound_kernel, grid, dim3(64), 0, c->stream, c->sub, c->s_pad, c->s, c->gb32, c->st32, c->tile32, c->gm32, c->stm32, c->gc32, d_c, b, A,
                        pl ? 0xe : 0xf, d_o);
     rh_dev<double> pl_gb;
     rh_dev<float> pl_tile32;
@@ -334,7 +341,7 @@
         RH_HIP(hipMemsetAsync(pl_gb, 0, sizeof(double) * 7 * (size_t)c->ng_pad, c->stream));
         RH_TRY(rhk_group_bounds_of(c, c->pl_sub, c->s_pad, c->s, c->ngroups, pl_gb, c->ng_pad));
         rhk_runs32_of(c, pl_gb, S4_TG, c->ntile, pl_tile32);
-        hipLaunchKernelGGL(cls_sound_kernel, grid, dim3(64), 0, c->stream, c->pl_sub, c->s_pad, c->s, c->pl_gb32, c->pl_st32, pl_tile32, c->pl_gm32, c->pl_stm32, d_c,
+        hipLaunchKernelGGL(cls_sound_kernel, grid, dim3(64), 0, c->stream, c->pl_sub, c->s_pad, c->s, c->pl_gb32, c->pl_st32, pl_tile32, c->pl_gm32, c->pl_stm32, c->pl_gc32, d_c,
                            b, A, 0x1, d_o);
     }
     RH_HIP(hipGetLastError());
@@ -358,6 +365,59 @@
 extern "C" int rh_dbg_cls_soundness_nsig(rh_cloud *c, const rh_shape *shapes, int32_t b, const rh_params *p, uint64_t *out)
 {
     return cls_soundness_run(c, shapes, b, p, out, 64, 4);
+}
+
+extern "C" int rh_dbg_cls_soundness_ncone(rh_cloud *c, const rh_shape *shapes, int32_t b, const rh_params *p, uint64_t *out)
+{
+    return cls_soundness_run(c, shapes, b, p, out, 68, 4);
+}
+
+extern "C" int rh_dbg_ncone(const double *normals, int32_t cnt, float *cone_out, const rh_shape *shapes, int32_t nshapes, const rh_params *p, double M,
+                            double Nm, double Ln, int f32, float *fields_out, int32_t *meet_out)
+{
+    if (cone_out == nullptr || cnt < 0 || cnt > 64 || nshapes < 0 || (nshapes > 0 && (shapes == nullptr || p == nullptr || meet_out == nullptr))) {
+        rh_set_error("rh_dbg_ncone: bad arguments");
+        return RH_E_INVALID;
+    }
+    if (normals != nullptr) {
+        double d[64][3], sx[64], sy[64], sz[64];
+        int dk[64], cn[64], inf[64];
+        for (int i = 0; i < 64; i++) {
+            d[i][0] = d[i][1] = d[i][2] = 0.0;
+            dk[i] = i < cnt ? ncone_dir(normals[3 * i], normals[3 * i + 1], normals[3 * i + 2], d[i]) : 0;
+            sx[i] = d[i][0]; sy[i] = d[i][1]; sz[i] = d[i][2];
+            cn[i] = dk[i] == 1 ? 1 : 0; inf[i] = dk[i] == 2 ? 1 : 0;
+        }
+        for (int off = 32; off > 0; off >>= 1)
+            for (int i = 0; i < off; i++) { sx[i] += sx[i + off]; sy[i] += sy[i + off]; sz[i] += sz[i + off]; cn[i] += cn[i + off]; inf[i] += inf[i + off]; }
+        double m[3];
+        const bool has_axis = ncone_axis(sx[0], sy[0], sz[0], cn[0], m);
+        double cmin = __builtin_inf();
+        for (int i = 0; i < 64; i++)
+            if (dk[i] == 1) cmin = fmin(cmin, (m[0] * d[i][0] + m[1] * d[i][1]) + m[2] * d[i][2]);
+        ncone_record(m, has_axis, cmin, cn[0], inf[0] != 0, cone_out);
+    }
+    const rh_f32x4 gc = { cone_out[0], cone_out[1], cone_out[2], cone_out[3] };
+    for (int32_t j = 0; j < nshapes; j++) {
+        Probe Q;
+        RH_TRY(probe_make("rh_dbg_ncone", "planes", 1 << RH_PLANE, shapes + j, p, M, Nm, Ln, f32, Q));
+        if (fields_out != nullptr)
+            for (int k = 0; k < 2; k++) fields_out[2 * j + k] = Q.box[8 + k];
+        meet_out[j] = ncone_meet(Q.box, gc) ? 1 : 0;
+    }
+    return RH_OK;
+}
+
+extern "C" int rh_dbg_ncones(rh_cloud *c, int which, float *out, int64_t cap, int64_t *ngroups_out)
+{
+    if (c == nullptr || ngroups_out == nullptr || cap < 0 || which < 0 || which > 1) { rh_set_error("rh_dbg_ncones: bad arguments"); return RH_E_INVALID; }
+    const float *src = which == 0 ? c->gc32.get() : c->pl_gc32.get();
+    *ngroups_out = src == nullptr || (which == 1 && c->pl_sub == nullptr) ? 0 : c->ngroups;
+    if (out == nullptr || *ngroups_out == 0 || cap < 4 * *ngroups_out) return RH_OK;
+    RH_HIP(hipSetDevice(c->device));
+    RH_HIP(hipMemcpyAsync(out, src, sizeof(float) * 4 * (size_t)c->ngroups, hipMemcpyDeviceToHost, c->stream));
+    RH_HIP(hipStreamSynchronize(c->stream));
+    return RH_OK;
 }
 
 extern "C" int rh_dbg_nsig(const rh_shape *shape, const rh_params *p, double M, double Nm, double Ln, int f32, uint32_t *mask_out,
diff --git a/ransac.jl_amd/csrc/score4_shared.h b/ransac.jl_amd/csrc/score4_shared.h
--- a/ransac.jl_amd/csrc/score4_shared.h
+++ b/ransac.jl_amd/csrc/score4_shared.h
@@ -18,13 +18,21 @@
     return (__builtin_bit_cast(uint32_t, v) & 0x7fffffffu) > 0x7f800000u;
 }
 
-template <int KIND> struct S4Fields { static constexpr int NBOX = KIND == RH_PLANE ? 8 : (KIND == RH_SPHERE ? 5 : (KIND == RH_CYLINDER ? 10 : 11)); };
+template <int KIND> struct S4Fields {
+    static constexpr int NBOX = KIND == RH_PLANE ? 10 : (KIND == RH_SPHERE ? 5 : (KIND == RH_CYLINDER ? 10 : 11));
+    static constexpr int NLIST = KIND == RH_PLANE ? 8 : NBOX;
+};
 
 static __device__ __forceinline__ bool nsig_meet(const float (&B)[rh4::RH_BOX_FIELDS], const rh_u32x4 gm)
 {
     return (((__builtin_bit_cast(uint32_t, B[5]) & gm.x) | (__builtin_bit_cast(uint32_t, B[6]) & gm.y)) | (__builtin_bit_cast(uint32_t, B[7]) & gm.z)) != 0u;
 }
 
+static __host__ __device__ __forceinline__ bool ncone_meet(const float (&B)[rh4::RH_BOX_FIELDS], const rh_f32x4 cone)
+{
+    return !(__builtin_fmaf(B[2], cone.z, __builtin_fmaf(B[1], cone.y, B[0] * cone.x)) < __builtin_fmaf(B[8], cone.w, -B[9]));
+}
+
 inline int cdiv4(int64_t a, int64_t b) { return (int)((a + b - 1) / b); }
 
 }
```

Measured after the change: 88.29 million candidates/s. About the same (-0.9%).
